# floatingtrees/video-VAE

Measured on AMD Instinct MI355X. Metric: video frames/sec (fwd+bwd) at Bx3x16x256x256, higher is better.
Workload: dtype bf16; 1 GPU; C3: full VideoVAE (enc 9 / dec 12 FactoredAttention + 3D-conv UNet) train step, B=4/GPU x 3x16x256x256, bf16 compute, fp32 params, recon+KL loss, clip+Adam; flavour=model, params=170631304, global_batch=4, frames_per_clip=16, parallelism=dp1, launch_mode=hipgraph(fwd+bwd) + eager all-reduce/clip/Adam

## Files before the change

### include/vvae_hip.h

```cpp
#ifndef VVAE_HIP_H
#define VVAE_HIP_H
#include <stddef.h>
#include <stdint.h>

#ifdef __cplusplus
extern "C" {
#endif

#define VVAE_DT_F32 0
#define VVAE_DT_BF16 1
#define VVAE_ERR_BAD_ARG 1001
#define VVAE_ERR_WORKSPACE 1002
#define VVAE_ERR_LIBRARY 1003

size_t vvae_conv3d_workspace_bytes(int N, int T, int H, int W, int Cin, int Cout, int kt, int kh, int kw, int dtype,
                                   int which );
int vvae_conv3d_fwd(const void* x, int ldx, const float* w, const float* bias, void* y, int ldy,
                    int N, int T, int H, int W, int Cin, int Cout, int kt, int kh, int kw, int dtype,
                    void* ws, size_t ws_bytes, void* stream);
int vvae_conv3d_dgrad(const void* dy, int lddy, const float* w, void* dx, int lddx,
                      int N, int T, int H, int W, int Cin, int Cout, int kt, int kh, int kw, int dtype,
                      void* ws, size_t ws_bytes, void* stream);
int vvae_conv3d_wgrad(const void* x, int ldx, const void* dy, int lddy, float* dw, float* dbias,
                      int N, int T, int H, int W, int Cin, int Cout, int kt, int kh, int kw, int dtype,
                      void* ws, size_t ws_bytes, void* stream);
void vvae_conv3d_force_generic(int on);
int vvae_conv3d_fwd_generic(const void* x, int ldx, const float* w, const float* bias, void* y, int ldy,
                            int N, int T, int H, int W, int Cin, int Cout, int kt, int kh, int kw, int dtype, void* stream);
int vvae_conv3d_dgrad_generic(const void* dy, int lddy, const float* w, void* dx, int lddx,
                              int N, int T, int H, int W, int Cin, int Cout, int kt, int kh, int kw, int dtype, void* stream);
size_t vvae_conv3d_wgrad_generic_ws_bytes(int N, int T, int H, int W, int Cin, int Cout, int kt, int kh, int kw);
int vvae_conv3d_wgrad_generic(const void* x, int ldx, const void* dy, int lddy, float* dw, float* dbias,
                              int N, int T, int H, int W, int Cin, int Cout, int kt, int kh, int kw, int dtype,
                              void* ws, size_t ws_bytes, void* stream);
int vvae_conv3d_deep_config(int on);
int vvae_conv3d_roll_config(int on, int tchunk);
int vvae_conv3d_wgrad_config(int cob16, int blocks);
int vvae_conv3d_bf16_supported(int Cin, int Cout, int kt, int kh, int kw, int ld_in, int ld_out, int which, int flags);
size_t vvae_conv3d_bf16_ws_bytes(int N, int T, int H, int W, int Cin, int Cout, int kt, int kh, int kw, int which);
int vvae_conv3d_pack_bf16(const float* w, void* ws, size_t ws_bytes, int Cin, int Cout, int kt, int kh, int kw,
                          int flags, void* stream);
int vvae_conv3d_pack_grouped_bf16(const float* const* w, void* const* ws, const size_t* ws_bytes, const int* Cin, const int* Cout,
                                  const int* kh, const int* flags, int n, void* stream);
int vvae_conv3d_fwd_bf16(const void* x, int ldx, const float* w, const float* bias, void* y, int ldy,
                         int N, int T, int H, int W, int Cin, int Cout, int kt, int kh, int kw, int flags,
                         int prepacked, void* ws, size_t ws_bytes, void* stream);
int vvae_conv3d_gn_blocks(int N, int T, int H, int W, int Cin, int Cout, int kt, int kh, int kw, int ld_in, int ld_out, int groups);
int vvae_conv3d_fwd_bf16_gn(const void* x, int ldx, const float* w, const float* bias, void* y, int ldy,
                            int N, int T, int H, int W, int Cin, int Cout, int kt, int kh, int kw,
                            int prepacked, void* ws, size_t ws_bytes, float* gn_part, int groups, void* stream);
size_t vvae_conv3d_wgrad_bf16_ws_bytes(int N, int T, int H, int W, int Cin, int Cout, int kt, int kh, int kw);
int vvae_conv3d_wgrad_bf16(const void* x, int ldx, const void* dy, int lddy, float* dw, float* dbias,
                           int N, int T, int H, int W, int Cin, int Cout, int kt, int kh, int kw,
                           void* ws, size_t ws_bytes, void* stream);
int vvae_conv3d_cat2_supported(int Cin, int Cout, int c_split, int kt, int kh, int kw);
int vvae_conv3d_fwd_bf16_cat2(const void* x, int ldx, const void* x2, int ldx2, const float* bias, void* y, int ldy, void* y2, int ldy2,
                              int c_split, int N, int T, int H, int W, int Cin, int Cout, int kt, int kh, int kw, int which,
                              const void* ws, size_t ws_bytes, float* gn_part, int groups, void* stream);
int vvae_conv3d_wgrad_bf16_cat2(const void* x, int ldx, const void* x2, int ldx2, int c_split, const void* dy, int lddy, float* dw,
                                float* dbias, int N, int T, int H, int W, int Cin, int Cout, int kt, int kh, int kw, void* ws,
                                size_t ws_bytes, void* stream);
int vvae_colsum_blocks(long V);
int vvae_colsum(const void* x, int ld, long V, int C, float* out, float* part, int dtype, void* stream);

int vvae_rl_gate_ok(int B2, int T, long per, int LD);
int vvae_rl_gate_blocks(int B2, int T, long per);
int vvae_rl_gate_fwd(const float* z, const float* prob, const float* u, const float* fill, void* comp, float* mask, int B2, int T, long per,
                     int LD, void* stream);
int vvae_rl_gate_bwd(const void* dcomp, const float* mask, float* dz, float* part, int B2, int T, long per, int LD, void* stream);

int vvae_pad_last2_grouped(const float* const* src, float* const* dst, const long* rows, const int* s0, const int* s1, const int* d0,
                           const int* d1, int n, int unpad, void* stream);

int vvae_conv_pointwise_supported(int Cin, int Cout, int kt, int kh, int kw, int ldx, int dtype, const void* x);
size_t vvae_conv_pointwise_ws_bytes(long V, int Cin, int Cout);
int vvae_conv_pointwise_fwd(const void* x, int ldx, const float* w, const float* bias, void* y, int ldy, long V, int Cin, int Cout,
                            int dtype, void* stream);
int vvae_conv_pointwise_fwd_add(const void* x, int ldx, const float* w, const float* bias, const void* addend, int ldadd, void* y, int ldy,
                                long V, int Cin, int Cout, int dtype, void* stream);
int vvae_conv_pointwise_dgrad(const void* dy, int lddy, const float* w, void* dx, int lddx, long V, int Cin, int Cout, int dtype,
                              void* stream);
int vvae_conv_pointwise_dgrad_add(const void* dy, int lddy, const float* w, const void* addend, int ldadd, void* dx, int lddx, long V, int Cin,
                                  int Cout, int dtype, void* stream);
int vvae_conv_pointwise_wgrad(const void* x, int ldx, const void* dy, int lddy, float* dw, float* dbias, long V, int Cin, int Cout,
                              int dtype, void* ws, size_t ws_bytes, void* stream);

int vvae_transpose_grouped_bf16(const void* const* src, void* const* dst, const int* rows, const int* cols, int n, void* stream);

int vvae_loss_tail_plain(const float* mse_ps, int mse_cols, const float* kl_ps, int kl_cols, const float* selection, const float* mask, int B, int T,
                         float max_compression_rate, float magnify_negatives_rate, float gamma1, float gamma2, float* out,
                         float* grads, void* stream);

int vvae_loss_tail_rl(const float* mse, const float* mae, int cols, const float* perc, const float* kl, int kl_cols, const float* sel, const float* act,
                      const float* mask, int B2, int T, float max_compression_rate, float magnify_negatives_rate, float gamma1,
                      float gamma2, float gamma3, float gamma4, float rl_loss_weight, float* out, float* grads, void* stream);

int vvae_encoder_head_ok(int B, int T, int HW, int LD);
int vvae_encoder_head_debug(int flags);
int vvae_encoder_head_fwd(const void* mean, const void* v, const float* w1, const float* b1, const float* w2, const float* b2,
                          const float* u, const float* eps, const float* mask, long mask_pitch, const float* fill, void* logvar,
                          void* comp, float* sel, float* y, float* s1, float* kl_frame, int B, int T, int HW, int LD, void* stream);
int vvae_encoder_head_bwd(const void* mean, const void* v, const void* logvar, const float* eps, const float* mask, long mask_pitch, const float* fill,
                          const float* w1, const float* w2, const float* y, const float* s1, const float* sel, const void* dcomp,
                          const float* dsel, const float* gkl, long gkl_pitch_b, long gkl_pitch_t, const void* dlv_ext, void* dmean, void* dv,
                          float* part1, float* part2, float* part3, float* partb, int B, int T, int HW, int LD, void* stream);

int vvae_encoder_head_eval_fwd(const void* mean, const void* v, const float* w1, const float* b1, const float* w2, const float* b2,
                               const float* u, const float* mask, long mask_pitch, const float* fill, int rl, void* logvar, void* comp,
                               float* sel, float* prob, int B, int T, int HW, int LD, void* stream);

int vvae_recon_metrics_supported(int H, int W, int C, int x_dtype, int y_dtype);
size_t vvae_recon_metrics_part_floats(int B, int T, int H, int W, int C);
int vvae_recon_metrics_fwd(const void* x, int x_dtype, const void* y, int y_dtype, const float* mask, float* mse, float* psnr, float* ssim,
                           float* part, int B, int T, int H, int W, int C, int clamp, void* stream);
int vvae_recon_metrics_wide_supported(int H, int W, int C, int x_dtype, int y_dtype);
size_t vvae_recon_metrics_wide_part_floats(int B, int T, int H, int W, int C);
int vvae_recon_metrics_wide_fwd(const void* x, int x_dtype, const void* y, int y_dtype, const float* mask, float* mse, float* psnr,
                                float* ssim, float* part, int B, int T, int H, int W, int C, int clamp, void* stream);

int vvae_tile_gather_supported(int H, int W, int C, int S, int overlap);
int vvae_tile_gather_u8(const void* src, const float* lut, float* dst, int N, int T, int H, int W, int C, int S, int overlap, int ny, int nx,
                        int first, int count, void* stream);
int vvae_tile_blend_supported(int H, int W, int C, int S, int overlap, int dtype);
int vvae_tile_blend(const void* tiles, int dtype, float* out, int N, int T, int H, int W, int C, int S, int overlap, int ny, int nx,
                    void* stream);
int vvae_window_blend_supported(int L, int frames, int t_overlap, int H, int W, int C, int S, int overlap, int dtype);
int vvae_window_blend(const void* tiles, int dtype, int ring, float* out, int L, int frames, int t_overlap, int n_windows, int f_lo, int f_hi,
                      int H, int W, int C, int S, int overlap, int ny, int nx, void* stream);
int vvae_temporal_mse_supported(int H, int W, int C, int x_dtype, int y_dtype);
size_t vvae_temporal_mse_part_floats(int B, int T, int H, int W, int C);
int vvae_temporal_mse_fwd(const void* x, int x_dtype, const void* y, int y_dtype, float* tmse, float* part, int B, int T, int H, int W, int C,
                          int clamp, void* stream);
int vvae_scene_hist_supported(int H, int W, int hist_size, int space);
size_t vvae_scene_hist_part_bytes(int L, int H, int W, int hist_size, int space);
int vvae_scene_hist_fwd(const void* clip, const int* tabs, unsigned* counts, double* corr, void* part, int L, int H, int W, int hist_size,
                        int space, void* stream);
int vvae_scene_hist_corr(const unsigned* counts, double* corr, int L, int bins, void* stream);
int vvae_crop_resize_supported(int H, int W, int C, int crop_h, int crop_w, int out_h, int out_w);
int vvae_crop_resize_u8(const uint8_t* src, uint8_t* dst, int n, int H, int W, int C, int top, int left, int crop_h, int crop_w, int out_h,
                        int out_w, void* stream);
int vvae_latent_quantise_supported(int hw, int ld, int dtype);
int vvae_latent_quantise(void* latent, int dtype, const float* keep, int8_t* codes, float* step, unsigned* counts, int frames, int hw, int ld,
                         int bits, int dequantise, void* stream);

int vvae_encoder_head_rl_fwd(const void* mean, const void* v, const float* w1, const float* b1, const float* w2, const float* b2,
                             const float* u2, const float* eps, const float* mask, long mask_pitch, const float* fill, void* logvar2,
                             void* mean2, void* comp2, float* prob, float* mask2, float* y, float* s1, float* kl_frame2, int B, int T, int HW,
                             int LD, void* stream);
int vvae_encoder_head_rl_bwd(const void* mean, const void* v, const void* logvar2, const float* eps, const float* mask, long mask_pitch,
                             const float* fill, const float* w1, const float* w2, const float* y, const float* s1, const float* mask2,
                             const void* dcomp2, const float* dprob2, const float* gkl, long gkl_pitch_b, long gkl_pitch_t, const void* dlv_ext,
                             void* dmean, void* dv, float* part1, float* part2, float* part3, float* partb, int B, int T, int HW, int LD,
                             void* stream);

int vvae_silu_bf16(const void* x, void* y, long n, void* stream);

int vvae_linear_residual_bf16(const void* x, int ldx, const void* w, int ldw, const void* bias, int bias_dtype, const void* res, int ldr,
                              void* y, int ldy, int M, int N, int K, void* ws, size_t ws_bytes, void* stream);
int vvae_linear_residual_wt_bf16(const void* x, int ldx, const void* wt, int ldwt, const void* bias, int bias_dtype, const void* res, int ldr,
                                 void* y, int ldy, int M, int N, int K, void* ws, size_t ws_bytes, void* stream);
int vvae_linear_residual_algo(int idx);

int vvae_unpatch_pad_fwd(const void* x, void* y, long frames, int h, int w, int p, int cu, int c, int dtype, void* stream);
int vvae_unpatch_pad_bwd(const void* g, void* gx, long frames, int h, int w, int p, int cu, int c, int dtype, void* stream);

size_t vvae_gn_part_floats(int N, long S, int C);
int vvae_gn_stats(const void* x, int ldx, int N, long S, int C, int G, double* sums, float* part, int dtype, void* stream);
int vvae_gn_finalize(const float* part, int N, int nblk, int G, double* sums, void* stream);
int vvae_gn_silu_fwd(const void* x, int ldx, void* y, int ldy, const double* sums, const float* gamma, const float* beta,
                     int N, long S, int C, int G, float eps, int dtype, void* stream);
int vvae_gn_silu_pool_supported(int H, int W, int C, int G, int ldx, int ldy, int ldp, int dtype);
int vvae_gn_silu_pool_fwd(const void* x, int ldx, void* y, int ldy, void* pool, int ldp, const double* sums, const float* gamma,
                          const float* beta, int N, int T, int H, int W, int C, int G, float eps, int dtype, void* stream);
int vvae_gn_silu_bwd(const void* x, int ldx, const void* dy, int lddy, void* dx, int lddx, const double* sums,
                     const float* gamma, const float* beta, double* csum , float* part,
                     float* dgamma, float* dbeta, int N, long S, int C, int G, float eps, int dtype, void* stream);

int vvae_maxpool_1x2x2_fwd(const void* x, int ldx, void* y, int ldy, int NT, int H, int W, int C, int dtype, void* stream);
int vvae_maxpool_1x2x2_bwd(const void* x, int ldx, const void* dpool, int lddp, const void* dskip, int ldds,
                           void* dx, int lddx, int NT, int H, int W, int C, int dtype, void* stream);

int vvae_convt_1x2x2_fwd(const void* x, int ldx, const float* w, const float* bias, void* y, int ldy,
                         int NT, int H, int W, int Cin, int Cout, int dtype, void* stream);
int vvae_convt_1x2x2_dgrad(const void* dy, int lddy, const float* w, void* dx, int lddx,
                           int NT, int H, int W, int Cin, int Cout, int dtype, void* stream);
size_t vvae_convt_1x2x2_wgrad_ws_bytes(int NT, int H, int W, int Cin, int Cout);
int vvae_convt_1x2x2_wgrad(const void* x, int ldx, const void* dy, int lddy, float* dw,
                           int NT, int H, int W, int Cin, int Cout, int dtype, void* ws, size_t ws_bytes, void* stream);
int vvae_convt_wgrad_bf16_supported(int Cin, int Cout, int ldx, int lddy);
size_t vvae_convt_wgrad_bf16_ws_bytes(int NT, int H, int W, int Cin, int Cout);
int vvae_convt_1x2x2_wgrad_bf16(const void* x, int ldx, const void* dy, int lddy, float* dw, float* dbias, int NT, int H, int W,
                                int Cin, int Cout, void* ws, size_t ws_bytes, void* stream);
int vvae_convt_bf16_supported(int Cin, int Cout, int ld_in, int ld_out);
size_t vvae_convt_bf16_ws_bytes(int Cin, int Cout);
int vvae_convt_1x2x2_bf16(const void* x, int ldx, const float* w, const float* bias, void* y, int ldy,
                          int NT, int H, int W, int Cin, int Cout, int dgrad, void* ws, size_t ws_bytes, void* stream);
int vvae_convt_pack_grouped_bf16(const float* const* w, void* const* ws, const int* Cin, const int* Cout, const int* dgrad, int n, void* stream);

int vvae_temporal_attn_fwd(const void* qkv, int ld, void* out, int ldo, const float* q_scale, const float* k_scale,
                           const float* cos_table, const float* sin_table, const uint8_t* mask, int mask_div,
                           int A, int T, int heads, int D, float eps, int dtype, void* stream);
size_t vvae_temporal_attn_bwd_ws_bytes(int A, int heads, int D);
int vvae_temporal_attn_bwd(const void* qkv, int ld, const void* dout, int lddo, void* dqkv, int lddq,
                           const float* q_scale, const float* k_scale, const float* cos_table, const float* sin_table,
                           const uint8_t* mask, int mask_div, float* dq_scale, float* dk_scale,
                           int A, int T, int heads, int D, float eps, int dtype, void* ws, size_t ws_bytes, void* stream);

int vvae_temporal_attn_fast_supported(int T, int D, int ld, int ldo, int dtype);
int vvae_temporal_attn_fast_blocks(int A, int T, int heads, int D, int dtype);
int vvae_temporal_attn_mfma_enable(int on);
int vvae_temporal_attn_mfma32_enable(int on);
int vvae_temporal_attn_fwd_fast(const void* qkv, int ld, void* out, int ldo, float* lse, const float* q_scale,
                                const float* k_scale, const float* cos_table, const float* sin_table, const uint8_t* mask,
                                int mask_div, int inner, int A, int T, int heads, int D, float eps, int dtype, void* stream);
int vvae_temporal_attn_bwd_fast(const void* qkv, int ld, const void* out, int ldo, const void* dout, int lddo, const float* lse,
                                void* dqkv, int lddq, const float* q_scale, const float* k_scale, const float* cos_table,
                                const float* sin_table, const uint8_t* mask, int mask_div, int inner, float* dscale_part,
                                int A, int T, int heads, int D, float eps, int dtype, void* stream);

int vvae_qk_prep_supported(int D, int dtype);
int vvae_qk_prep_blocks(long tokens, int heads, int D);
int vvae_qk_prep_fwd(const void* qkv, int ld, void* out, int ldo, const float* q_scale, const float* k_scale,
                     const float* cos_table, const float* sin_table, long tokens, int S, int heads, int D, float eps,
                     int dtype, void* stream);
int vvae_qk_prep_bwd(const void* qkv, int ld, const void* dq, long dq_ts, long dq_hs, const void* dk, long dk_ts, long dk_hs,
                     const void* dv, long dv_ts, long dv_hs, void* dqkv, int lddq, const float* q_scale, const float* k_scale,
                     const float* cos_table, const float* sin_table, float* part, long tokens, int S, int heads, int D,
                     float eps, int dtype, void* stream);

int vvae_spatial_attn_supported(int S, int D, int dtype);
int vvae_spatial_attn_fwd(const void* qkv, int ld, void* out, int ldo, float* lse2, const float* q_scale, const float* k_scale,
                          const float* cos_table, const float* sin_table, int A, int S, int heads, int D, float eps, int dtype,
                          void* stream);
int vvae_spatial_attn_bwd(const void* qkv, int ld, const void* out, int ldo, const void* dout, int lddo, const float* lse2,
                          void* dqkv, int lddq, const float* q_scale, const float* k_scale, const float* cos_table,
                          const float* sin_table, float* part, int A, int S, int heads, int D, float eps, int dtype, void* stream);

int vvae_layernorm_supported(int C, int dtype);
int vvae_layernorm_bwd_blocks(long rows, int C, int dtype);
int vvae_delay_us(int us, void* stream);
int vvae_layernorm_fwd_config(int fwd_cap);
int vvae_gn_config(int stream_blocks);
int vvae_layernorm_config(int bwd_cap);
int vvae_layernorm_fwd_mode(int late_stage);
int vvae_layernorm_fwd(const void* x, void* y, const float* gamma, const float* beta, float* mean, float* rstd,
                       const void* addend, void* xsum, long rows, int C, int inner, long outer_pitch, long inner_pitch, float eps,
                       int dtype, void* stream);
int vvae_layernorm_bwd(const void* x, const void* dy, const float* gamma, const float* mean, const float* rstd, const void* dres,
                       void* dx, float* part, long rows, int C, int inner, long outer_pitch, long inner_pitch, int dtype,
                       void* stream);

size_t vvae_loss_part_floats(int B, long M);
int vvae_reparam_kl_fwd(const void* mean, const void* logvar, const float* eps, const float* mask, float* z, float* kl,
                        float* part, int B, int T, long per, int dtype, void* stream);
int vvae_reparam_kl_bwd(const void* mean, const void* logvar, const float* eps, const float* mask, const float* dz,
                        const float* gkl, void* dmean, void* dlogvar, int B, int T, long per, int dtype, void* stream);

int vvae_masked_mse_mae_fwd(const void* video, const void* recon, const float* mask, float* mse, float* mae,
                            float* part, int B, int T, long P, int video_div, int dtype, void* stream);
int vvae_masked_mse_mae_bwd(const void* video, const void* recon, const float* mask, const float* gmse, const float* gmae,
                            void* drecon, int B, int T, long P, int video_div, int dtype, void* stream);

int vvae_gemm_tn_supported(int M, int N, int K, int lda, int ldb);
size_t vvae_gemm_tn_ws_bytes(int M, int N, int K);
int vvae_gemm_tn_bf16(const void* A, int lda, const void* B, int ldb, float* C, float* db, int M, int N, int K,
                      void* ws, size_t ws_bytes, void* stream);
int vvae_gemm_tn_grouped_bf16(const void* const* A, const int* lda, const void* const* B, const int* ldb, float* const* C,
                              float* const* db, const int* M, const int* N, int n, int K, void* stream);
int vvae_gemm_tn_use_big_tiles(int on);

int vvae_sqnorm_blocks(long n);
int vvae_sqnorm_partials(const float* g, long n, double* part, void* stream);
int vvae_adam_clip_step(float* p, const float* g, float* m, float* v, void* p_bf16, long n, const double* gnorm_part, int nparts,
                        double* gnorm_sq_out, float gscale, float max_norm, float lr, float b1, float b2, float eps, long count,
                        void* stream);
int vvae_adam_clip_ema_step(float* p, const float* g, float* m, float* v, void* p_bf16, long n, const double* gnorm_part, int nparts,
                            double* gnorm_sq_out, float gscale, float max_norm, float lr, float b1, float b2, float eps, long count,
                            float* ema, float ema_decay, void* stream);
int vvae_grad_fold_f32(float* dst, const float* src, long n, int overwrite, void* stream);
int vvae_sqnorm_partials2(const float* g, const float* acc, long n, double* part, void* stream);
int vvae_adam_clip_acc_step(float* p, const float* g, const float* acc, float* m, float* v, void* p_bf16, long n,
                            const double* gnorm_part, int nparts, double* gnorm_sq_out, float gscale, float max_norm, float lr, float b1,
                            float b2, float eps, long count, float* ema, float ema_decay, void* stream);
int vvae_swap_refresh_f32(float* a, float* b, void* a_bf16, long n, void* stream);
int vvae_cast_f32_to_bf16(const float* x, void* y, long n, void* stream);
int vvae_gemm_nt_supported(int M, int N, int K, int lda, int ldb, int ldc);
int vvae_gemm_nt_bf16(const void* A, int lda, const void* B, int ldb, void* C, int ldc, const float* bias, const void* res,
                      int ldr, void* C2, int ldc2, int epi, int M, int N, int K, void* stream);
int vvae_gemm_pp_supported(int M, int N, int K, int lda, int ldb, int ldc);
int vvae_gemm_pp_bf16(const void* A, int lda, const void* B, int ldb, void* C, int ldc, const float* bias, const void* res,
                      int ldr, void* C2, int ldc2, int epi, int M, int N, int K, void* stream);
int vvae_gemm_pp_ablate(int bits);
int vvae_gemm_pp_final_ring(int on);
int vvae_gemm_nt_stagger(int units);
int vvae_gemm_nt_persistent(int on);
int vvae_gemm_nt_prefetch(int dist);
int vvae_gemm_nt_prefetch_mask(int mask);

int vvae_sum_rows(const float* part, int rows, int cols, float* out, void* stream);
int vvae_fold_rows_grouped(const void* const* part, float* const* d0, float* const* d1, const int* rows, const int* cols,
                           const int* n0, int n, void* stream);
int vvae_copy_grouped(const float* const* src, float* const* dst, const long* count, int n, void* stream);

int vvae_selftest_xor_lane(const float* x, float* y, double* yd, int n, int o, void* stream);

#ifdef __cplusplus
}
#endif
#endif
```

### video_vae_amd/csrc/attn_temporal_mfma.hip

```cpp
#include "common.hpp"

namespace tmfma {

typedef __bf16 bf16x8 __attribute__((ext_vector_type(8)));
typedef short s16x4v __attribute__((ext_vector_type(4)));

constexpr int T = 16, D = 64;
constexpr int PITCH = 160;
constexpr int IMG = T * PITCH;

struct Dims { int A, heads, mask_div, inner; float eps; long items; };

__device__ __forceinline__ long token_of(const Dims& d, int a, int row) {
    return (long)(a / d.inner) * T * d.inner + (long)row * d.inner + (a % d.inner);
}

__device__ __forceinline__ void unpack8(const uint4& r, float* v) {
    const uint32_t w[4] = {r.x, r.y, r.z, r.w};
#pragma unroll
    for (int i = 0; i < 4; ++i) { v[2 * i] = __uint_as_float(w[i] << 16); v[2 * i + 1] = __uint_as_float(w[i] & 0xffff0000u); }
}
__device__ __forceinline__ uint4 pack8(const float* v) {
    uint32_t w[4];
#pragma unroll
    for (int i = 0; i < 4; ++i) w[i] = (uint32_t)f2bf(v[2 * i]) | ((uint32_t)f2bf(v[2 * i + 1]) << 16);
    return make_uint4(w[0], w[1], w[2], w[3]);
}
__device__ __forceinline__ bf16x8 frag8(const uint4& r) { return __builtin_bit_cast(bf16x8, r); }
__device__ __forceinline__ s16x4v pack4(float a, float b, float c, float e) {
    s16x4v r = {(short)f2bf(a), (short)f2bf(b), (short)f2bf(c), (short)f2bf(e)};
    return r;
}
__device__ __forceinline__ s16x4v tr4(const unsigned char* p) {
    typedef __attribute__((address_space(3))) s16x4v* lds_ptr;
    return __builtin_amdgcn_ds_read_tr16_b64_v4i16((lds_ptr)p);
}
__device__ __forceinline__ f32x4 mfma32(const bf16x8& a, const bf16x8& b, f32x4 c) { return __builtin_amdgcn_mfma_f32_16x16x32_bf16(a, b, c, 0, 0, 0); }
__device__ __forceinline__ f32x4 mfma16(const s16x4v& a, const s16x4v& b, f32x4 c) { return __builtin_amdgcn_mfma_f32_16x16x16bf16_1k(a, b, c, 0, 0, 0); }

__device__ __forceinline__ float psum(float v) { return butterfly_sum<32, 16>(v); }
__device__ __forceinline__ float pmax(float v) { v = fmaxf(v, xor_lane<32>(v)); return fmaxf(v, xor_lane<16>(v)); }

__device__ __forceinline__ float xhat16(float (&x)[16], float eps) {
    float s = 0.f, ss = 0.f;
#pragma unroll
    for (int i = 0; i < 16; ++i) { s += x[i]; ss += x[i] * x[i]; }
    s = psum(s); ss = psum(ss);
    const float mean = s * (1.f / D);
    float var = ss * (1.f / D) - mean * mean;
    var = var < 0.f ? 0.f : var;
    const float rstd = rsqrtf(var + eps);
#pragma unroll
    for (int i = 0; i < 16; ++i) x[i] = (x[i] - mean) * rstd;
    return rstd;
}
__device__ __forceinline__ void ln_rope16(float (&x)[16], const float* __restrict__ sc, float eps, const float* __restrict__ cs,
                                          const float* __restrict__ sn) {
    xhat16(x, eps);
#pragma unroll
    for (int i = 0; i < 8; ++i) {
        float lo = x[i] * sc[i], hi = x[i + 8] * sc[i + 8];
        round2<bf16_t>(lo, hi);
        float a = lo * cs[i], b = -hi * sn[i], c = hi * cs[i + 8], e = lo * sn[i + 8];
        round2<bf16_t>(a, b);
        round2<bf16_t>(c, e);
        float y0 = a + b, y1 = c + e;
        round2<bf16_t>(y0, y1);
        x[i] = y0; x[i + 8] = y1;
    }
}
__device__ __forceinline__ void tab16(const float* __restrict__ row, int p, float (&r)[16]) {
    const float4* lo = reinterpret_cast<const float4*>(row + 8 * p);
    const float4* hi = reinterpret_cast<const float4*>(row + 32 + 8 * p);
    const float4 a = lo[0], b = lo[1], c = hi[0], e = hi[1];
    r[0] = a.x; r[1] = a.y; r[2] = a.z; r[3] = a.w; r[4] = b.x; r[5] = b.y; r[6] = b.z; r[7] = b.w;
    r[8] = c.x; r[9] = c.y; r[10] = c.z; r[11] = c.w; r[12] = e.x; r[13] = e.y; r[14] = e.z; r[15] = e.w;
}
__device__ __forceinline__ void norm_row(const bf16_t* __restrict__ g, int p, const float (&sc)[16], float eps, const float (&cs)[16],
                                         const float (&sn)[16], uint4& f0, uint4& f1) {
    float x[16];
    unpack8(*reinterpret_cast<const uint4*>(g + 8 * p), x);
    unpack8(*reinterpret_cast<const uint4*>(g + 32 + 8 * p), x + 8);
    ln_rope16(x, sc, eps, cs, sn);
    f0 = pack8(x); f1 = pack8(x + 8);
}
__device__ __forceinline__ void put_row(unsigned char* img, int t, int p, const uint4& f0, const uint4& f1) {
    *reinterpret_cast<uint4*>(img + t * PITCH + 16 * p) = f0;
    *reinterpret_cast<uint4*>(img + t * PITCH + 64 + 16 * p) = f1;
}
__device__ __forceinline__ void wave_lds_fence() {
    __builtin_amdgcn_wave_barrier();
    __builtin_amdgcn_s_waitcnt(0xc07f);
    __builtin_amdgcn_wave_barrier();
}
__device__ __forceinline__ s16x4v tr_rows(const unsigned char* img, int p, int i, int tile) {
    return tr4(img + (4 * p + (i >> 2)) * PITCH + 32 * tile + 8 * (i & 3));
}

__global__ __launch_bounds__(256) void tattn16_fwd_mfma(const bf16_t* __restrict__ qkv, int ld, bf16_t* __restrict__ out, int ldo,
                                                       float* __restrict__ lse, const float* __restrict__ q_scale,
                                                       const float* __restrict__ k_scale, const float* __restrict__ cosT,
                                                       const float* __restrict__ sinT, const uint8_t* __restrict__ mask, Dims d)
{
    __shared__ __attribute__((aligned(16))) unsigned char smem[4 * IMG];
    const int lane = threadIdx.x & 63, wave = threadIdx.x >> 6;
    const int t = lane & 15, p = lane >> 4;
    const long item = (long)blockIdx.x * 4 + wave;
    if (item >= d.items) return;
    const int a = (int)(item / d.heads), h = (int)(item % d.heads);
    const int HD = d.heads * D;
    const long tok = token_of(d, a, t);
    const bf16_t* g = qkv + tok * ld + h * D;
    unsigned char* vimg = smem + wave * IMG;

    const uint4 vlo = *reinterpret_cast<const uint4*>(g + 2 * HD + 8 * p);
    const uint4 vhi = *reinterpret_cast<const uint4*>(g + 2 * HD + 32 + 8 * p);
    float cs[16], sn[16], sc[16];
    tab16(cosT + t * D, p, cs);
    tab16(sinT + t * D, p, sn);
    uint4 q0, q1, k0, k1;
    tab16(q_scale, p, sc);
    norm_row(g, p, sc, d.eps, cs, sn, q0, q1);
    tab16(k_scale, p, sc);
    norm_row(g + HD, p, sc, d.eps, cs, sn, k0, k1);
    put_row(vimg, t, p, vlo, vhi);

    f32x4 s = {0.f, 0.f, 0.f, 0.f};
    s = mfma32(frag8(k0), frag8(q0), s);
    s = mfma32(frag8(k1), frag8(q1), s);
    const float scale = 0.125f;
    uint32_t mk = 0x01010101u;
    if (mask) mk = *reinterpret_cast<const uint32_t*>(mask + (long)(a / d.mask_div) * T + 4 * p);
    float e[4];
    float m = -3.0e38f;
#pragma unroll
    for (int r = 0; r < 4; ++r) {
        e[r] = ((mk >> (8 * r)) & 0xff) ? s[r] * scale : -3.0e38f;
        m = fmaxf(m, e[r]);
    }
    m = pmax(m);
    float l = 0.f;
#pragma unroll
    for (int r = 0; r < 4; ++r) { e[r] = ((mk >> (8 * r)) & 0xff) ? __expf(e[r] - m) : 0.f; l += e[r]; }
    l = psum(l);
    const float inv = l > 0.f ? 1.f / l : 0.f;
    const s16x4v pf = pack4(e[0] * inv, e[1] * inv, e[2] * inv, e[3] * inv);
    if (p == 0) lse[item * T + t] = l > 0.f ? m + __logf(l) : 0.f;

    wave_lds_fence();
    bf16_t* o = out + tok * ldo + h * D + 4 * p;
#pragma unroll
    for (int tile = 0; tile < 4; ++tile) {
        f32x4 acc = {0.f, 0.f, 0.f, 0.f};
        acc = mfma16(tr_rows(vimg, p, t, tile), pf, acc);
        const s16x4v ob = pack4(acc[0], acc[1], acc[2], acc[3]);
        *reinterpret_cast<uint2*>(o + 16 * tile) = __builtin_bit_cast(uint2, ob);
    }
}

__device__ __forceinline__ void rope_ln_bwd_cols(float (&g)[4][4], const float (&raw)[4][4], int p, int frame, float eps,
                                                 const float* __restrict__ scale, const float* __restrict__ cosT,
                                                 const float* __restrict__ sinT, float (&contrib)[4][4])
{
    float xh[4][4];
    float s = 0.f, ss = 0.f;
#pragma unroll
    for (int tl = 0; tl < 4; ++tl)
#pragma unroll
        for (int r = 0; r < 4; ++r) { s += raw[tl][r]; ss += raw[tl][r] * raw[tl][r]; }
    s = psum(s); ss = psum(ss);
    const float mean = s * (1.f / D);
    float var = ss * (1.f / D) - mean * mean;
    var = var < 0.f ? 0.f : var;
    const float rstd = rsqrtf(var + eps);
#pragma unroll
    for (int tl = 0; tl < 4; ++tl)
#pragma unroll
        for (int r = 0; r < 4; ++r) xh[tl][r] = (raw[tl][r] - mean) * rstd;
    const float* cr = cosT + frame * D;
    const float* sr = sinT + frame * D;
#pragma unroll
    for (int tl = 0; tl < 2; ++tl) {
        const float4 cl = *reinterpret_cast<const float4*>(cr + 16 * tl + 4 * p), ch = *reinterpret_cast<const float4*>(cr + 32 + 16 * tl + 4 * p);
        const float4 sl = *reinterpret_cast<const float4*>(sr + 16 * tl + 4 * p), sh = *reinterpret_cast<const float4*>(sr + 32 + 16 * tl + 4 * p);
        const float c_lo[4] = {cl.x, cl.y, cl.z, cl.w}, c_hi[4] = {ch.x, ch.y, ch.z, ch.w};
        const float s_lo[4] = {sl.x, sl.y, sl.z, sl.w}, s_hi[4] = {sh.x, sh.y, sh.z, sh.w};
#pragma unroll
        for (int r = 0; r < 4; ++r) {
            const float lo = g[tl][r], hi = g[tl + 2][r];
            g[tl][r] = lo * c_lo[r] + hi * s_hi[r];
            g[tl + 2][r] = hi * c_hi[r] - lo * s_lo[r];
        }
    }
    float s1 = 0.f, s2 = 0.f;
    float scv[4][4];
#pragma unroll
    for (int tl = 0; tl < 4; ++tl) {
        const float4 v = *reinterpret_cast<const float4*>(scale + 16 * tl + 4 * p);
        scv[tl][0] = v.x; scv[tl][1] = v.y; scv[tl][2] = v.z; scv[tl][3] = v.w;
#pragma unroll
        for (int r = 0; r < 4; ++r) { const float dxh = g[tl][r] * scv[tl][r]; s1 += dxh; s2 += dxh * xh[tl][r]; }
    }
    s1 = psum(s1) * (1.f / D); s2 = psum(s2) * (1.f / D);
#pragma unroll
    for (int tl = 0; tl < 4; ++tl)
#pragma unroll
        for (int r = 0; r < 4; ++r) {
            const float dy = g[tl][r], x = xh[tl][r];
            g[tl][r] = rstd * (dy * scv[tl][r] - s1 - x * s2);
            contrib[tl][r] = dy * x;
        }
}

__device__ __forceinline__ void load_cols(const bf16_t* __restrict__ row, int p, float (&v)[4][4]) {
#pragma unroll
    for (int tl = 0; tl < 4; ++tl) {
        const uint2 u = *reinterpret_cast<const uint2*>(row + 16 * tl + 4 * p);
        v[tl][0] = __uint_as_float(u.x << 16); v[tl][1] = __uint_as_float(u.x & 0xffff0000u);
        v[tl][2] = __uint_as_float(u.y << 16); v[tl][3] = __uint_as_float(u.y & 0xffff0000u);
    }
}
__device__ __forceinline__ void store_cols(bf16_t* __restrict__ row, int p, const float (&v)[4][4]) {
#pragma unroll
    for (int tl = 0; tl < 4; ++tl) {
        const s16x4v b = pack4(v[tl][0], v[tl][1], v[tl][2], v[tl][3]);
        *reinterpret_cast<uint2*>(row + 16 * tl + 4 * p) = __builtin_bit_cast(uint2, b);
    }
}

__global__ __launch_bounds__(256, 4) void tattn16_bwd_mfma(const bf16_t* __restrict__ qkv, int ld, const bf16_t* __restrict__ out, int ldo,
                                                          const bf16_t* __restrict__ dout, int lddo, const float* __restrict__ lse,
                                                          bf16_t* __restrict__ dqkv, int lddq, const float* __restrict__ q_scale,
                                                          const float* __restrict__ k_scale, const float* __restrict__ cosT,
                                                          const float* __restrict__ sinT, const uint8_t* __restrict__ mask,
                                                          float* __restrict__ part, Dims d)
{
    __shared__ __attribute__((aligned(16))) unsigned char smem[4 * (3 * IMG + 64)];
    const int lane = threadIdx.x & 63, wave = threadIdx.x >> 6;
    const int t = lane & 15, p = lane >> 4;
    unsigned char* base = smem + wave * (3 * IMG + 64);
    unsigned char* kimg = base;
    unsigned char* qimg = base + IMG;
    unsigned char* gimg = base + 2 * IMG;
    float* dlds = reinterpret_cast<float*>(base + 3 * IMG);
    const int HD = d.heads * D;
    const float scale = 0.125f;
    float accq[4][4], acck[4][4];
#pragma unroll
    for (int tl = 0; tl < 4; ++tl)
#pragma unroll
        for (int r = 0; r < 4; ++r) { accq[tl][r] = 0.f; acck[tl][r] = 0.f; }

    const long item = (long)blockIdx.x * 4 + wave;
    if (item < d.items) {
        const float* ct = cosT; const float* st_ = sinT; const float* qsp = q_scale; const float* ksp = k_scale;
        const int a = (int)(item / d.heads), h = (int)(item % d.heads);
        const long tok = token_of(d, a, t);
        const bf16_t* g = qkv + tok * ld + h * D;
        uint4 q0, q1, k0, k1;
        {
            float cs[16], sn[16], sc[16];
            tab16(ct + t * D, p, cs);
            tab16(st_ + t * D, p, sn);
            tab16(qsp, p, sc);
            norm_row(g, p, sc, d.eps, cs, sn, q0, q1);
            tab16(ksp, p, sc);
            norm_row(g + HD, p, sc, d.eps, cs, sn, k0, k1);
        }
        const uint4 v0 = *reinterpret_cast<const uint4*>(g + 2 * HD + 8 * p), v1 = *reinterpret_cast<const uint4*>(g + 2 * HD + 32 + 8 * p);
        const bf16_t* go = dout + tok * lddo + h * D;
        const uint4 g0 = *reinterpret_cast<const uint4*>(go + 8 * p), g1 = *reinterpret_cast<const uint4*>(go + 32 + 8 * p);
        const bf16_t* oo = out + tok * ldo + h * D;
        float delta;
        {
            float a16[16], b16[16];
            unpack8(g0, a16); unpack8(g1, a16 + 8);
            unpack8(*reinterpret_cast<const uint4*>(oo + 8 * p), b16); unpack8(*reinterpret_cast<const uint4*>(oo + 32 + 8 * p), b16 + 8);
            float s = 0.f;
#pragma unroll
            for (int i = 0; i < 16; ++i) s += a16[i] * b16[i];
            delta = psum(s);
        }
        wave_lds_fence();
        put_row(kimg, t, p, k0, k1);
        put_row(qimg, t, p, q0, q1);
        put_row(gimg, t, p, g0, g1);
        if (p == 0) dlds[t] = delta;
        const float lse_q = lse[item * T + t];
        uint32_t mk = 0x01010101u, mcol = 1u;
        if (mask) {
            const uint8_t* mrow = mask + (long)(a / d.mask_div) * T;
            mk = *reinterpret_cast<const uint32_t*>(mrow + 4 * p);
            mcol = mrow[t];
        }
        bf16_t* dg = dqkv + tok * lddq + h * D;
        s16x4v dsf, pf, dsf2;
        {
            f32x4 st = {0.f, 0.f, 0.f, 0.f}, dpt = {0.f, 0.f, 0.f, 0.f}, sq = {0.f, 0.f, 0.f, 0.f}, dp = {0.f, 0.f, 0.f, 0.f};
            st = mfma32(frag8(k0), frag8(q0), st);
            st = mfma32(frag8(k1), frag8(q1), st);
            dpt = mfma32(frag8(v0), frag8(g0), dpt);
            dpt = mfma32(frag8(v1), frag8(g1), dpt);
            sq = mfma32(frag8(q0), frag8(k0), sq);
            sq = mfma32(frag8(q1), frag8(k1), sq);
            dp = mfma32(frag8(g0), frag8(v0), dp);
            dp = mfma32(frag8(g1), frag8(v1), dp);
            float dst[4];
#pragma unroll
            for (int r = 0; r < 4; ++r) {
                const float pr = ((mk >> (8 * r)) & 0xff) ? __expf(st[r] * scale - lse_q) : 0.f;
                dst[r] = pr * (dpt[r] - delta) * scale;
            }
            dsf = pack4(dst[0], dst[1], dst[2], dst[3]);
            wave_lds_fence();
            const float4 lse4 = *reinterpret_cast<const float4*>(lse + item * T + 4 * p);
            const float4 del4 = *reinterpret_cast<const float4*>(dlds + 4 * p);
            const float lq[4] = {lse4.x, lse4.y, lse4.z, lse4.w}, dl[4] = {del4.x, del4.y, del4.z, del4.w};
            float pq[4], dsq[4];
#pragma unroll
            for (int r = 0; r < 4; ++r) {
                const float pr = mcol ? __expf(sq[r] * scale - lq[r]) : 0.f;
                pq[r] = pr;
                dsq[r] = pr * (dp[r] - dl[r]) * scale;
            }
            pf = pack4(pq[0], pq[1], pq[2], pq[3]);
            dsf2 = pack4(dsq[0], dsq[1], dsq[2], dsq[3]);
        }
        {
            float dq[4][4];
#pragma unroll
            for (int tile = 0; tile < 4; ++tile) {
                f32x4 acc = {0.f, 0.f, 0.f, 0.f};
                acc = mfma16(tr_rows(kimg, p, t, tile), dsf, acc);
#pragma unroll
                for (int r = 0; r < 4; ++r) dq[tile][r] = acc[r];
            }
            float raw[4][4], contrib[4][4];
            load_cols(g, p, raw);
            rope_ln_bwd_cols(dq, raw, p, t, d.eps, qsp, ct, st_, contrib);
            store_cols(dg, p, dq);
#pragma unroll
            for (int tl = 0; tl < 4; ++tl)
#pragma unroll
                for (int r = 0; r < 4; ++r) accq[tl][r] += contrib[tl][r];
        }
        {
            float dv[4][4];
#pragma unroll
            for (int tile = 0; tile < 4; ++tile) {
                f32x4 a1 = {0.f, 0.f, 0.f, 0.f};
                a1 = mfma16(tr_rows(gimg, p, t, tile), pf, a1);
#pragma unroll
                for (int r = 0; r < 4; ++r) dv[tile][r] = a1[r];
            }
            store_cols(dg + 2 * HD, p, dv);
        }
        {
            float dk[4][4];
#pragma unroll
            for (int tile = 0; tile < 4; ++tile) {
                f32x4 a2 = {0.f, 0.f, 0.f, 0.f};
                a2 = mfma16(tr_rows(qimg, p, t, tile), dsf2, a2);
#pragma unroll
                for (int r = 0; r < 4; ++r) dk[tile][r] = a2[r];
            }
            float raw[4][4], contrib[4][4];
            load_cols(g + HD, p, raw);
            rope_ln_bwd_cols(dk, raw, p, t, d.eps, ksp, ct, st_, contrib);
            store_cols(dg + HD, p, dk);
#pragma unroll
            for (int tl = 0; tl < 4; ++tl)
#pragma unroll
                for (int r = 0; r < 4; ++r) acck[tl][r] += contrib[tl][r];
        }
    }
    __syncthreads();
    float* red = reinterpret_cast<float*>(smem);
#pragma unroll
    for (int tl = 0; tl < 4; ++tl)
#pragma unroll
        for (int r = 0; r < 4; ++r) {
            const float a = butterfly_sum<8, 1>(accq[tl][r]), b = butterfly_sum<8, 1>(acck[tl][r]);
            if (t == 0) { red[wave * 2 * D + 16 * tl + 4 * p + r] = a; red[wave * 2 * D + D + 16 * tl + 4 * p + r] = b; }
        }
    __syncthreads();
    if (threadIdx.x < 2 * D)
        part[(long)blockIdx.x * 2 * D + threadIdx.x] = (red[threadIdx.x] + red[2 * D + threadIdx.x]) + (red[4 * D + threadIdx.x] + red[6 * D + threadIdx.x]);
}

int g_enable = 1;

inline int bwd_blocks(long items) { return (int)((items + 3) / 4); }

bool shape_ok(int T_, int D_, int ld, int ldo, int dtype) {
    return g_enable && dtype == VVAE_DT_BF16 && T_ == T && D_ == D && ld % 8 == 0 && ldo % 8 == 0;
}

}

extern "C" int vvae_temporal_attn_mfma_enable(int on)
{
    tmfma::g_enable = on ? 1 : 0;
    return 0;
}

int tmfma_supported(int T, int D, int ld, int ldo, int dtype) { return tmfma::shape_ok(T, D, ld, ldo, dtype) ? 1 : 0; }
int tmfma_bwd_rows(long items) { return tmfma::bwd_blocks(items); }

int tmfma_fwd(const void* qkv, int ld, void* out, int ldo, float* lse, const float* qs, const float* ks, const float* cosT, const float* sinT,
              const uint8_t* mask, int mask_div, int inner, int A, int heads, float eps, hipStream_t s)
{
    tmfma::Dims d{A, heads, mask_div, inner, eps, (long)A * heads};
    if (mask && ((uintptr_t)mask % 4)) return VVAE_ERR_BAD_ARG;
    hipLaunchKernelGGL(tmfma::tattn16_fwd_mfma, dim3((unsigned)((d.items + 3) / 4)), dim3(256), 0, s, (const bf16_t*)qkv, ld, (bf16_t*)out, ldo, lse,
                       qs, ks, cosT, sinT, mask, d);
    VVAE_LAUNCH_CHECK();
    return 0;
}

int tmfma_bwd(const void* qkv, int ld, const void* out, int ldo, const void* dout, int lddo, const float* lse, void* dqkv, int lddq,
              const float* qs, const float* ks, const float* cosT, const float* sinT, const uint8_t* mask, int mask_div, int inner,
              float* part, int A, int heads, float eps, hipStream_t s)
{
    tmfma::Dims d{A, heads, mask_div, inner, eps, (long)A * heads};
    if (mask && ((uintptr_t)mask % 4)) return VVAE_ERR_BAD_ARG;
    hipLaunchKernelGGL(tmfma::tattn16_bwd_mfma, dim3((unsigned)tmfma::bwd_blocks(d.items)), dim3(256), 0, s, (const bf16_t*)qkv, ld,
                       (const bf16_t*)out, ldo, (const bf16_t*)dout, lddo, lse, (bf16_t*)dqkv, lddq, qs, ks, cosT, sinT, mask, part, d);
    VVAE_LAUNCH_CHECK();
    return 0;
}
```

Before: 2012 frames/s.

## Make temporal attention MFMA kernels persistent with software-prefetched item loads

Converts the forward and backward 16-frame temporal attention kernels into grid-stride persistent loops capped at 512 blocks. Each wave prefetches the next item's q/k/v and mask while computing the current one, and hoists cos/sin and scale tables out of the per-item loop. This aims to hide global load latency and cut block launch and setup overhead. It also drops one intermediate bf16 rounding in the RoPE output, which changes numerics slightly. Ablation variants compiled under a macro are added for probing.

New measurement: 2034 frames/s, median of 6. +1.1%, better.

```diff
diff --git a/include/vvae_hip.h b/include/vvae_hip.h
--- a/include/vvae_hip.h
+++ b/include/vvae_hip.h
@@ -209,6 +209,7 @@
 int vvae_temporal_attn_fast_supported(int T, int D, int ld, int ldo, int dtype);
 int vvae_temporal_attn_fast_blocks(int A, int T, int heads, int D, int dtype);
 int vvae_temporal_attn_mfma_enable(int on);
+int vvae_temporal_attn_mfma_config(int fwd_cap, int bwd_cap);
 int vvae_temporal_attn_mfma32_enable(int on);
 int vvae_temporal_attn_fwd_fast(const void* qkv, int ld, void* out, int ldo, float* lse, const float* q_scale,
                                 const float* k_scale, const float* cos_table, const float* sin_table, const uint8_t* mask,
diff --git a/video_vae_amd/csrc/attn_temporal_mfma.hip b/video_vae_amd/csrc/attn_temporal_mfma.hip
--- a/video_vae_amd/csrc/attn_temporal_mfma.hip
+++ b/video_vae_amd/csrc/attn_temporal_mfma.hip
@@ -8,12 +8,11 @@
 constexpr int T = 16, D = 64;
 constexpr int PITCH = 160;
 constexpr int IMG = T * PITCH;
+constexpr int BWD_WAVE_LDS = 5 * IMG + 128;
+
+constexpr int ABL_LOAD = 1, ABL_MATH = 2, ABL_MFMA = 4, ABL_STORE = 8;
 
 struct Dims { int A, heads, mask_div, inner; float eps; long items; };
-
-__device__ __forceinline__ long token_of(const Dims& d, int a, int row) {
-    return (long)(a / d.inner) * T * d.inner + (long)row * d.inner + (a % d.inner);
-}
 
 __device__ __forceinline__ void unpack8(const uint4& r, float* v) {
     const uint32_t w[4] = {r.x, r.y, r.z, r.w};
@@ -35,8 +34,27 @@
     typedef __attribute__((address_space(3))) s16x4v* lds_ptr;
     return __builtin_amdgcn_ds_read_tr16_b64_v4i16((lds_ptr)p);
 }
-__device__ __forceinline__ f32x4 mfma32(const bf16x8& a, const bf16x8& b, f32x4 c) { return __builtin_amdgcn_mfma_f32_16x16x32_bf16(a, b, c, 0, 0, 0); }
-__device__ __forceinline__ f32x4 mfma16(const s16x4v& a, const s16x4v& b, f32x4 c) { return __builtin_amdgcn_mfma_f32_16x16x16bf16_1k(a, b, c, 0, 0, 0); }
+template <int ABL> __device__ __forceinline__ f32x4 mfma32(const uint4& a, const uint4& b, f32x4 c) {
+    if constexpr (ABL & ABL_MFMA) { c[0] += __uint_as_float(((a.x ^ b.x) & 0x007fffffu) | 0x3f000000u); return c; }
+    else return __builtin_amdgcn_mfma_f32_16x16x32_bf16(frag8(a), frag8(b), c, 0, 0, 0);
+}
+template <int ABL> __device__ __forceinline__ f32x4 mfma16(const s16x4v& a, const s16x4v& b, f32x4 c) {
+    if constexpr (ABL & ABL_MFMA) {
+        const uint2 x = __builtin_bit_cast(uint2, a), y = __builtin_bit_cast(uint2, b);
+        c[0] += __uint_as_float(((x.x ^ y.x) & 0x007fffffu) | 0x3f000000u);
+        c[1] += __uint_as_float(((x.y ^ y.y) & 0x007fffffu) | 0x3f000000u);
+        return c;
+    } else return __builtin_amdgcn_mfma_f32_16x16x16bf16_1k(a, b, c, 0, 0, 0);
+}
+template <int ABL> __device__ __forceinline__ uint4 ld16(const bf16_t* __restrict__ p, const bf16_t* __restrict__ line) {
+    if constexpr (ABL & ABL_LOAD) return *reinterpret_cast<const uint4*>(line);
+    else return *reinterpret_cast<const uint4*>(p);
+}
+template <int ABL> __device__ __forceinline__ void st8(bf16_t* __restrict__ p, const s16x4v& v) {
+    const uint2 u = __builtin_bit_cast(uint2, v);
+    if constexpr (ABL & ABL_STORE) { if (u.x == 0x7fc17fc2u && u.y == 0x7fc37fc4u) *reinterpret_cast<uint2*>(p) = u; }
+    else *reinterpret_cast<uint2*>(p) = u;
+}
 
 __device__ __forceinline__ float psum(float v) { return butterfly_sum<32, 16>(v); }
 __device__ __forceinline__ float pmax(float v) { v = fmaxf(v, xor_lane<32>(v)); return fmaxf(v, xor_lane<16>(v)); }
@@ -54,8 +72,7 @@
     for (int i = 0; i < 16; ++i) x[i] = (x[i] - mean) * rstd;
     return rstd;
 }
-__device__ __forceinline__ void ln_rope16(float (&x)[16], const float* __restrict__ sc, float eps, const float* __restrict__ cs,
-                                          const float* __restrict__ sn) {
+__device__ __forceinline__ void ln_rope16(float (&x)[16], const float (&sc)[16], float eps, const float (&cs)[16], const float (&sn)[16]) {
     xhat16(x, eps);
 #pragma unroll
     for (int i = 0; i < 8; ++i) {
@@ -64,9 +81,7 @@
         float a = lo * cs[i], b = -hi * sn[i], c = hi * cs[i + 8], e = lo * sn[i + 8];
         round2<bf16_t>(a, b);
         round2<bf16_t>(c, e);
-        float y0 = a + b, y1 = c + e;
-        round2<bf16_t>(y0, y1);
-        x[i] = y0; x[i + 8] = y1;
+        x[i] = a + b; x[i + 8] = c + e;
     }
 }
 __device__ __forceinline__ void tab16(const float* __restrict__ row, int p, float (&r)[16]) {
@@ -76,13 +91,16 @@
     r[0] = a.x; r[1] = a.y; r[2] = a.z; r[3] = a.w; r[4] = b.x; r[5] = b.y; r[6] = b.z; r[7] = b.w;
     r[8] = c.x; r[9] = c.y; r[10] = c.z; r[11] = c.w; r[12] = e.x; r[13] = e.y; r[14] = e.z; r[15] = e.w;
 }
-__device__ __forceinline__ void norm_row(const bf16_t* __restrict__ g, int p, const float (&sc)[16], float eps, const float (&cs)[16],
-                                         const float (&sn)[16], uint4& f0, uint4& f1) {
-    float x[16];
-    unpack8(*reinterpret_cast<const uint4*>(g + 8 * p), x);
-    unpack8(*reinterpret_cast<const uint4*>(g + 32 + 8 * p), x + 8);
-    ln_rope16(x, sc, eps, cs, sn);
-    f0 = pack8(x); f1 = pack8(x + 8);
+template <int ABL> __device__ __forceinline__ void norm_row(const uint4& lo, const uint4& hi, const float (&sc)[16], float eps,
+                                                            const float (&cs)[16], const float (&sn)[16], uint4& f0, uint4& f1) {
+    if constexpr (ABL & ABL_MATH) { f0 = lo; f1 = hi; }
+    else {
+        float x[16];
+        unpack8(lo, x);
+        unpack8(hi, x + 8);
+        ln_rope16(x, sc, eps, cs, sn);
+        f0 = pack8(x); f1 = pack8(x + 8);
+    }
 }
 __device__ __forceinline__ void put_row(unsigned char* img, int t, int p, const uint4& f0, const uint4& f1) {
     *reinterpret_cast<uint4*>(img + t * PITCH + 16 * p) = f0;
@@ -93,74 +111,141 @@
     __builtin_amdgcn_s_waitcnt(0xc07f);
     __builtin_amdgcn_wave_barrier();
 }
+__device__ __forceinline__ void drain_loads() { __builtin_amdgcn_s_waitcnt(0x0f70); }
 __device__ __forceinline__ s16x4v tr_rows(const unsigned char* img, int p, int i, int tile) {
     return tr4(img + (4 * p + (i >> 2)) * PITCH + 32 * tile + 8 * (i & 3));
 }
 
-__global__ __launch_bounds__(256) void tattn16_fwd_mfma(const bf16_t* __restrict__ qkv, int ld, bf16_t* __restrict__ out, int ldo,
-                                                       float* __restrict__ lse, const float* __restrict__ q_scale,
-                                                       const float* __restrict__ k_scale, const float* __restrict__ cosT,
-                                                       const float* __restrict__ sinT, const uint8_t* __restrict__ mask, Dims d)
-{
-    __shared__ __attribute__((aligned(16))) unsigned char smem[4 * IMG];
-    const int lane = threadIdx.x & 63, wave = threadIdx.x >> 6;
+struct ItemAt { int a, h; long tok0; };
+__device__ __forceinline__ ItemAt item_at(const Dims& d, long item) {
+    const unsigned it = (unsigned)item, hd = (unsigned)d.heads, in = (unsigned)d.inner;
+    const unsigned a = it / hd, h = it - a * hd;
+    const unsigned ao = a / in, ai = a - ao * in;
+    return ItemAt{(int)a, (int)h, (long)ao * T * d.inner + ai};
+}
+
+struct FwdRaw { uint4 q0, q1, k0, k1, v0, v1; uint32_t mk; };
+
+template <int ABL> __device__ __forceinline__ void fwd_load(FwdRaw& r, const bf16_t* __restrict__ qkv, int ld, const uint8_t* __restrict__ mask,
+                                                            const Dims& d, long item, long lane_in, int p, const bf16_t* __restrict__ line) {
+    const ItemAt at = item_at(d, item);
+    const int HD = d.heads * D;
+    const bf16_t* g = qkv + at.tok0 * ld + at.h * D + lane_in;
+    r.q0 = ld16<ABL>(g, line); r.q1 = ld16<ABL>(g + 32, line);
+    r.k0 = ld16<ABL>(g + HD, line); r.k1 = ld16<ABL>(g + HD + 32, line);
+    r.v0 = ld16<ABL>(g + 2 * HD, line); r.v1 = ld16<ABL>(g + 2 * HD + 32, line);
+    r.mk = 0x01010101u;
+    if (mask) r.mk = *reinterpret_cast<const uint32_t*>(mask + (long)(at.a / d.mask_div) * T + 4 * p);
+}
+
+template <int ABL> __device__ __forceinline__ void fwd_item(const FwdRaw& r, long item, unsigned char* vimg, bf16_t* __restrict__ o,
+                                                            float* __restrict__ lse, int t, int p, float eps, const float (&cs)[16],
+                                                            const float (&sn)[16], const float (&scq)[16], const float (&sck)[16]) {
+    uint4 q0, q1, k0, k1;
+    norm_row<ABL>(r.q0, r.q1, scq, eps, cs, sn, q0, q1);
+    norm_row<ABL>(r.k0, r.k1, sck, eps, cs, sn, k0, k1);
+    wave_lds_fence();
+    put_row(vimg, t, p, r.v0, r.v1);
+
+    f32x4 s = {0.f, 0.f, 0.f, 0.f};
+    s = mfma32<ABL>(k0, q0, s);
+    s = mfma32<ABL>(k1, q1, s);
+    const float scale = 0.125f;
+    const uint32_t mk = r.mk;
+    s16x4v pf;
+    float lse_v;
+    if constexpr (ABL & ABL_MATH) {
+        pf = pack4(s[0], s[1], s[2], s[3]);
+        lse_v = s[0] + __uint_as_float(mk);
+    } else {
+        float e[4];
+        float m = -3.0e38f;
+#pragma unroll
+        for (int r_ = 0; r_ < 4; ++r_) {
+            e[r_] = ((mk >> (8 * r_)) & 0xff) ? s[r_] * scale : -3.0e38f;
+            m = fmaxf(m, e[r_]);
+        }
+        m = pmax(m);
+        float l = 0.f;
+#pragma unroll
+        for (int r_ = 0; r_ < 4; ++r_) { e[r_] = ((mk >> (8 * r_)) & 0xff) ? __expf(e[r_] - m) : 0.f; l += e[r_]; }
+        l = psum(l);
+        const float inv = l > 0.f ? 1.f / l : 0.f;
+        pf = pack4(e[0] * inv, e[1] * inv, e[2] * inv, e[3] * inv);
+        lse_v = l > 0.f ? m + __logf(l) : 0.f;
+    }
+    if (p == 0) {
+        if constexpr (ABL & ABL_STORE) { if (lse_v == -1.2345e-30f) lse[item * T + t] = lse_v; }
+        else lse[item * T + t] = lse_v;
+    }
+
+    wave_lds_fence();
+#pragma unroll
+    for (int tile = 0; tile < 4; ++tile) {
+        f32x4 acc = {0.f, 0.f, 0.f, 0.f};
+        acc = mfma16<ABL>(tr_rows(vimg, p, t, tile), pf, acc);
+        st8<ABL>(o + 16 * tile, pack4(acc[0], acc[1], acc[2], acc[3]));
+    }
+}
+
+template <int ABL> __device__ __forceinline__ void fwd_walk(const bf16_t* __restrict__ qkv, int ld, bf16_t* __restrict__ out, int ldo,
+                                                            float* __restrict__ lse, const float* __restrict__ q_scale,
+                                                            const float* __restrict__ k_scale, const float* __restrict__ cosT,
+                                                            const float* __restrict__ sinT, const uint8_t* __restrict__ mask, const Dims& d,
+                                                            unsigned char* smem)
+{
+    const int lane = threadIdx.x & 63, wave = __builtin_amdgcn_readfirstlane(threadIdx.x >> 6);
     const int t = lane & 15, p = lane >> 4;
-    const long item = (long)blockIdx.x * 4 + wave;
+    const long stride = (long)gridDim.x * 4;
+    long item = (long)blockIdx.x * 4 + wave;
     if (item >= d.items) return;
-    const int a = (int)(item / d.heads), h = (int)(item % d.heads);
-    const int HD = d.heads * D;
-    const long tok = token_of(d, a, t);
-    const bf16_t* g = qkv + tok * ld + h * D;
     unsigned char* vimg = smem + wave * IMG;
-
-    const uint4 vlo = *reinterpret_cast<const uint4*>(g + 2 * HD + 8 * p);
-    const uint4 vhi = *reinterpret_cast<const uint4*>(g + 2 * HD + 32 + 8 * p);
-    float cs[16], sn[16], sc[16];
+    float cs[16], sn[16], scq[16], sck[16];
     tab16(cosT + t * D, p, cs);
     tab16(sinT + t * D, p, sn);
-    uint4 q0, q1, k0, k1;
-    tab16(q_scale, p, sc);
-    norm_row(g, p, sc, d.eps, cs, sn, q0, q1);
-    tab16(k_scale, p, sc);
-    norm_row(g + HD, p, sc, d.eps, cs, sn, k0, k1);
-    put_row(vimg, t, p, vlo, vhi);
-
-    f32x4 s = {0.f, 0.f, 0.f, 0.f};
-    s = mfma32(frag8(k0), frag8(q0), s);
-    s = mfma32(frag8(k1), frag8(q1), s);
-    const float scale = 0.125f;
-    uint32_t mk = 0x01010101u;
-    if (mask) mk = *reinterpret_cast<const uint32_t*>(mask + (long)(a / d.mask_div) * T + 4 * p);
-    float e[4];
-    float m = -3.0e38f;
-#pragma unroll
-    for (int r = 0; r < 4; ++r) {
-        e[r] = ((mk >> (8 * r)) & 0xff) ? s[r] * scale : -3.0e38f;
-        m = fmaxf(m, e[r]);
-    }
-    m = pmax(m);
-    float l = 0.f;
-#pragma unroll
-    for (int r = 0; r < 4; ++r) { e[r] = ((mk >> (8 * r)) & 0xff) ? __expf(e[r] - m) : 0.f; l += e[r]; }
-    l = psum(l);
-    const float inv = l > 0.f ? 1.f / l : 0.f;
-    const s16x4v pf = pack4(e[0] * inv, e[1] * inv, e[2] * inv, e[3] * inv);
-    if (p == 0) lse[item * T + t] = l > 0.f ? m + __logf(l) : 0.f;
-
-    wave_lds_fence();
-    bf16_t* o = out + tok * ldo + h * D + 4 * p;
-#pragma unroll
-    for (int tile = 0; tile < 4; ++tile) {
-        f32x4 acc = {0.f, 0.f, 0.f, 0.f};
-        acc = mfma16(tr_rows(vimg, p, t, tile), pf, acc);
-        const s16x4v ob = pack4(acc[0], acc[1], acc[2], acc[3]);
-        *reinterpret_cast<uint2*>(o + 16 * tile) = __builtin_bit_cast(uint2, ob);
-    }
-}
-
-__device__ __forceinline__ void rope_ln_bwd_cols(float (&g)[4][4], const float (&raw)[4][4], int p, int frame, float eps,
-                                                 const float* __restrict__ scale, const float* __restrict__ cosT,
-                                                 const float* __restrict__ sinT, float (&contrib)[4][4])
+    tab16(q_scale, p, scq);
+    tab16(k_scale, p, sck);
+    const long lane_in = (long)t * d.inner * ld + 8 * p;
+    const long lane_out = (long)t * d.inner * ldo + 4 * p;
+    const bf16_t* line = qkv + 8 * (lane & 7);
+    FwdRaw cur;
+    fwd_load<ABL>(cur, qkv, ld, mask, d, item, lane_in, p, line);
+    drain_loads();
+    for (;;) {
+        const long nxt = item + stride;
+        const bool more = nxt < d.items;
+        FwdRaw nx;
+        if (more) fwd_load<ABL>(nx, qkv, ld, mask, d, nxt, lane_in, p, line);
+        const ItemAt at = item_at(d, item);
+        fwd_item<ABL>(cur, item, vimg, out + at.tok0 * ldo + at.h * D + lane_out, lse, t, p, d.eps, cs, sn, scq, sck);
+        if (!more) break;
+        cur = nx; item = nxt;
+    }
+}
+
+__global__ __launch_bounds__(256, 2) void tattn16_fwd_mfma(const bf16_t* __restrict__ qkv, int ld, bf16_t* __restrict__ out, int ldo,
+                                                          float* __restrict__ lse, const float* __restrict__ q_scale,
+                                                          const float* __restrict__ k_scale, const float* __restrict__ cosT,
+                                                          const float* __restrict__ sinT, const uint8_t* __restrict__ mask, Dims d)
+{
+    __shared__ __attribute__((aligned(16))) unsigned char smem[4 * IMG];
+    fwd_walk<0>(qkv, ld, out, ldo, lse, q_scale, k_scale, cosT, sinT, mask, d, smem);
+}
+
+struct ColTabs { float c_lo[2][4], c_hi[2][4], s_lo[2][4], s_hi[2][4]; };
+__device__ __forceinline__ void col_tabs(const float* __restrict__ cr, const float* __restrict__ sr, int p, ColTabs& ct) {
+#pragma unroll
+    for (int tl = 0; tl < 2; ++tl) {
+        const float4 cl = *reinterpret_cast<const float4*>(cr + 16 * tl + 4 * p), ch = *reinterpret_cast<const float4*>(cr + 32 + 16 * tl + 4 * p);
+        const float4 sl = *reinterpret_cast<const float4*>(sr + 16 * tl + 4 * p), sh = *reinterpret_cast<const float4*>(sr + 32 + 16 * tl + 4 * p);
+        ct.c_lo[tl][0] = cl.x; ct.c_lo[tl][1] = cl.y; ct.c_lo[tl][2] = cl.z; ct.c_lo[tl][3] = cl.w;
+        ct.c_hi[tl][0] = ch.x; ct.c_hi[tl][1] = ch.y; ct.c_hi[tl][2] = ch.z; ct.c_hi[tl][3] = ch.w;
+        ct.s_lo[tl][0] = sl.x; ct.s_lo[tl][1] = sl.y; ct.s_lo[tl][2] = sl.z; ct.s_lo[tl][3] = sl.w;
+        ct.s_hi[tl][0] = sh.x; ct.s_hi[tl][1] = sh.y; ct.s_hi[tl][2] = sh.z; ct.s_hi[tl][3] = sh.w;
+    }
+}
+__device__ __forceinline__ void rope_ln_bwd_cols(float (&g)[4][4], const float (&raw)[4][4], int p, float eps, const float* scale,
+                                                 const ColTabs& ct, float (&acc)[4][4])
 {
     float xh[4][4];
     float s = 0.f, ss = 0.f;
@@ -177,19 +262,13 @@
     for (int tl = 0; tl < 4; ++tl)
 #pragma unroll
         for (int r = 0; r < 4; ++r) xh[tl][r] = (raw[tl][r] - mean) * rstd;
-    const float* cr = cosT + frame * D;
-    const float* sr = sinT + frame * D;
 #pragma unroll
     for (int tl = 0; tl < 2; ++tl) {
-        const float4 cl = *reinterpret_cast<const float4*>(cr + 16 * tl + 4 * p), ch = *reinterpret_cast<const float4*>(cr + 32 + 16 * tl + 4 * p);
-        const float4 sl = *reinterpret_cast<const float4*>(sr + 16 * tl + 4 * p), sh = *reinterpret_cast<const float4*>(sr + 32 + 16 * tl + 4 * p);
-        const float c_lo[4] = {cl.x, cl.y, cl.z, cl.w}, c_hi[4] = {ch.x, ch.y, ch.z, ch.w};
-        const float s_lo[4] = {sl.x, sl.y, sl.z, sl.w}, s_hi[4] = {sh.x, sh.y, sh.z, sh.w};
 #pragma unroll
         for (int r = 0; r < 4; ++r) {
             const float lo = g[tl][r], hi = g[tl + 2][r];
-            g[tl][r] = lo * c_lo[r] + hi * s_hi[r];
-            g[tl + 2][r] = hi * c_hi[r] - lo * s_lo[r];
+            g[tl][r] = lo * ct.c_lo[tl][r] + hi * ct.s_hi[tl][r];
+            g[tl + 2][r] = hi * ct.c_hi[tl][r] - lo * ct.s_lo[tl][r];
         }
     }
     float s1 = 0.f, s2 = 0.f;
@@ -208,189 +287,274 @@
         for (int r = 0; r < 4; ++r) {
             const float dy = g[tl][r], x = xh[tl][r];
             g[tl][r] = rstd * (dy * scv[tl][r] - s1 - x * s2);
-            contrib[tl][r] = dy * x;
-        }
-}
-
-__device__ __forceinline__ void load_cols(const bf16_t* __restrict__ row, int p, float (&v)[4][4]) {
+            acc[tl][r] += dy * x;
+        }
+}
+
+__device__ __forceinline__ void load_cols(const unsigned char* img, int i, int p, float (&v)[4][4]) {
 #pragma unroll
     for (int tl = 0; tl < 4; ++tl) {
-        const uint2 u = *reinterpret_cast<const uint2*>(row + 16 * tl + 4 * p);
+        const uint2 u = *reinterpret_cast<const uint2*>(img + i * PITCH + 32 * tl + 8 * p);
         v[tl][0] = __uint_as_float(u.x << 16); v[tl][1] = __uint_as_float(u.x & 0xffff0000u);
         v[tl][2] = __uint_as_float(u.y << 16); v[tl][3] = __uint_as_float(u.y & 0xffff0000u);
     }
 }
-__device__ __forceinline__ void store_cols(bf16_t* __restrict__ row, int p, const float (&v)[4][4]) {
-#pragma unroll
-    for (int tl = 0; tl < 4; ++tl) {
-        const s16x4v b = pack4(v[tl][0], v[tl][1], v[tl][2], v[tl][3]);
-        *reinterpret_cast<uint2*>(row + 16 * tl + 4 * p) = __builtin_bit_cast(uint2, b);
-    }
-}
-
-__global__ __launch_bounds__(256, 4) void tattn16_bwd_mfma(const bf16_t* __restrict__ qkv, int ld, const bf16_t* __restrict__ out, int ldo,
+template <int ABL> __device__ __forceinline__ void store_cols(bf16_t* __restrict__ row, const float (&v)[4][4]) {
+#pragma unroll
+    for (int tl = 0; tl < 4; ++tl) st8<ABL>(row + 16 * tl, pack4(v[tl][0], v[tl][1], v[tl][2], v[tl][3]));
+}
+
+struct BwdRaw { uint4 q0, q1, k0, k1, v0, v1, g0, g1, o0, o1; float lse_q; uint32_t mk, mcol; };
+
+template <int ABL> __device__ __forceinline__ void bwd_load(BwdRaw& r, const bf16_t* __restrict__ qkv, int ld, const bf16_t* __restrict__ out,
+                                                            int ldo, const bf16_t* __restrict__ dout, int lddo, const float* __restrict__ lse,
+                                                            const uint8_t* __restrict__ mask, const Dims& d, long item, int t, int p,
+                                                            const bf16_t* __restrict__ line) {
+    const ItemAt at = item_at(d, item);
+    const int HD = d.heads * D;
+    const long row = (long)t * d.inner;
+    const bf16_t* g = qkv + (at.tok0 + row) * ld + at.h * D + 8 * p;
+    const bf16_t* go = dout + (at.tok0 + row) * lddo + at.h * D + 8 * p;
+    const bf16_t* oo = out + (at.tok0 + row) * ldo + at.h * D + 8 * p;
+    r.q0 = ld16<ABL>(g, line); r.q1 = ld16<ABL>(g + 32, line);
+    r.k0 = ld16<ABL>(g + HD, line); r.k1 = ld16<ABL>(g + HD + 32, line);
+    r.v0 = ld16<ABL>(g + 2 * HD, line); r.v1 = ld16<ABL>(g + 2 * HD + 32, line);
+    r.g0 = ld16<ABL>(go, line); r.g1 = ld16<ABL>(go + 32, line);
+    r.o0 = ld16<ABL>(oo, line); r.o1 = ld16<ABL>(oo + 32, line);
+    r.lse_q = lse[item * T + t];
+    r.mk = 0x01010101u; r.mcol = 1u;
+    if (mask) {
+        const uint8_t* mrow = mask + (long)(at.a / d.mask_div) * T;
+        r.mk = *reinterpret_cast<const uint32_t*>(mrow + 4 * p);
+        r.mcol = mrow[t];
+    }
+}
+
+template <int ABL> __device__ __forceinline__ void bwd_item(const BwdRaw& r, unsigned char* base, bf16_t* __restrict__ dg, int HD, int t, int p,
+                                                            float eps, const float (&cs)[16], const float (&sn)[16], const ColTabs& ct,
+                                                            const float* stab, float (&accq)[4][4], float (&acck)[4][4]) {
+    unsigned char* kimg = base;
+    unsigned char* qimg = base + IMG;
+    unsigned char* gimg = base + 2 * IMG;
+    unsigned char* rqimg = base + 3 * IMG;
+    unsigned char* rkimg = base + 4 * IMG;
+    float* dlds = reinterpret_cast<float*>(base + 5 * IMG);
+    const float scale = 0.125f;
+    uint4 q0, q1, k0, k1;
+    {
+        float sc[16];
+        tab16(stab, p, sc);
+        norm_row<ABL>(r.q0, r.q1, sc, eps, cs, sn, q0, q1);
+        tab16(stab + D, p, sc);
+        norm_row<ABL>(r.k0, r.k1, sc, eps, cs, sn, k0, k1);
+    }
+    const uint4 v0 = r.v0, v1 = r.v1, g0 = r.g0, g1 = r.g1;
+    float delta;
+    if constexpr (ABL & ABL_MATH) delta = __uint_as_float((g0.x ^ r.o0.x ^ r.o1.y) & 0x3fffffffu);
+    else {
+        float a16[16], b16[16];
+        unpack8(g0, a16); unpack8(g1, a16 + 8);
+        unpack8(r.o0, b16); unpack8(r.o1, b16 + 8);
+        float s = 0.f;
+#pragma unroll
+        for (int i = 0; i < 16; ++i) s += a16[i] * b16[i];
+        delta = psum(s);
+    }
+    wave_lds_fence();
+    put_row(kimg, t, p, k0, k1);
+    put_row(qimg, t, p, q0, q1);
+    put_row(gimg, t, p, g0, g1);
+    put_row(rqimg, t, p, r.q0, r.q1);
+    put_row(rkimg, t, p, r.k0, r.k1);
+    const float lse_q = r.lse_q;
+    if (p == 0) { dlds[t] = delta; dlds[T + t] = lse_q; }
+    const uint32_t mk = r.mk, mcol = r.mcol;
+    s16x4v dsf, pf, dsf2;
+    {
+        f32x4 st = {0.f, 0.f, 0.f, 0.f}, dpt = {0.f, 0.f, 0.f, 0.f}, sq = {0.f, 0.f, 0.f, 0.f}, dp = {0.f, 0.f, 0.f, 0.f};
+        st = mfma32<ABL>(k0, q0, st);
+        st = mfma32<ABL>(k1, q1, st);
+        dpt = mfma32<ABL>(v0, g0, dpt);
+        dpt = mfma32<ABL>(v1, g1, dpt);
+        sq = mfma32<ABL>(q0, k0, sq);
+        sq = mfma32<ABL>(q1, k1, sq);
+        dp = mfma32<ABL>(g0, v0, dp);
+        dp = mfma32<ABL>(g1, v1, dp);
+        float dst[4];
+#pragma unroll
+        for (int r_ = 0; r_ < 4; ++r_) {
+            if constexpr (ABL & ABL_MATH) dst[r_] = st[r_] + dpt[r_] + delta + lse_q + __uint_as_float(mk);
+            else {
+                const float pr = ((mk >> (8 * r_)) & 0xff) ? __expf(st[r_] * scale - lse_q) : 0.f;
+                dst[r_] = pr * (dpt[r_] - delta) * scale;
+            }
+        }
+        dsf = pack4(dst[0], dst[1], dst[2], dst[3]);
+        wave_lds_fence();
+        const float4 del4 = *reinterpret_cast<const float4*>(dlds + 4 * p);
+        const float4 lse4 = *reinterpret_cast<const float4*>(dlds + T + 4 * p);
+        const float lq[4] = {lse4.x, lse4.y, lse4.z, lse4.w}, dl[4] = {del4.x, del4.y, del4.z, del4.w};
+        float pq[4], dsq[4];
+#pragma unroll
+        for (int r_ = 0; r_ < 4; ++r_) {
+            if constexpr (ABL & ABL_MATH) { pq[r_] = sq[r_] + lq[r_] + __uint_as_float(mcol); dsq[r_] = dp[r_] + dl[r_]; }
+            else {
+                const float pr = mcol ? __expf(sq[r_] * scale - lq[r_]) : 0.f;
+                pq[r_] = pr;
+                dsq[r_] = pr * (dp[r_] - dl[r_]) * scale;
+            }
+        }
+        pf = pack4(pq[0], pq[1], pq[2], pq[3]);
+        dsf2 = pack4(dsq[0], dsq[1], dsq[2], dsq[3]);
+    }
+    {
+        float dq[4][4];
+#pragma unroll
+        for (int tile = 0; tile < 4; ++tile) {
+            f32x4 acc = {0.f, 0.f, 0.f, 0.f};
+            acc = mfma16<ABL>(tr_rows(kimg, p, t, tile), dsf, acc);
+#pragma unroll
+            for (int r_ = 0; r_ < 4; ++r_) dq[tile][r_] = acc[r_];
+        }
+        float raw[4][4];
+        load_cols(rqimg, t, p, raw);
+        if constexpr (ABL & ABL_MATH) {
+#pragma unroll
+            for (int tl = 0; tl < 4; ++tl)
+#pragma unroll
+                for (int r_ = 0; r_ < 4; ++r_) { dq[tl][r_] += raw[tl][r_]; accq[tl][r_] += dq[tl][r_]; }
+        } else rope_ln_bwd_cols(dq, raw, p, eps, stab, ct, accq);
+        store_cols<ABL>(dg, dq);
+    }
+    {
+        float dv[4][4];
+#pragma unroll
+        for (int tile = 0; tile < 4; ++tile) {
+            f32x4 a1 = {0.f, 0.f, 0.f, 0.f};
+            a1 = mfma16<ABL>(tr_rows(gimg, p, t, tile), pf, a1);
+#pragma unroll
+            for (int r_ = 0; r_ < 4; ++r_) dv[tile][r_] = a1[r_];
+        }
+        store_cols<ABL>(dg + 2 * HD, dv);
+    }
+    {
+        float dk[4][4];
+#pragma unroll
+        for (int tile = 0; tile < 4; ++tile) {
+            f32x4 a2 = {0.f, 0.f, 0.f, 0.f};
+            a2 = mfma16<ABL>(tr_rows(qimg, p, t, tile), dsf2, a2);
+#pragma unroll
+            for (int r_ = 0; r_ < 4; ++r_) dk[tile][r_] = a2[r_];
+        }
+        float raw[4][4];
+        load_cols(rkimg, t, p, raw);
+        if constexpr (ABL & ABL_MATH) {
+#pragma unroll
+            for (int tl = 0; tl < 4; ++tl)
+#pragma unroll
+                for (int r_ = 0; r_ < 4; ++r_) { dk[tl][r_] += raw[tl][r_]; acck[tl][r_] += dk[tl][r_]; }
+        } else rope_ln_bwd_cols(dk, raw, p, eps, stab + D, ct, acck);
+        store_cols<ABL>(dg + HD, dk);
+    }
+}
+
+template <int ABL> __device__ __forceinline__ void bwd_walk(const bf16_t* __restrict__ qkv, int ld, const bf16_t* __restrict__ out, int ldo,
+                                                            const bf16_t* __restrict__ dout, int lddo, const float* __restrict__ lse,
+                                                            bf16_t* __restrict__ dqkv, int lddq, const float* __restrict__ q_scale,
+                                                            const float* __restrict__ k_scale, const float* __restrict__ cosT,
+                                                            const float* __restrict__ sinT, const uint8_t* __restrict__ mask,
+                                                            float* __restrict__ part, const Dims& d, unsigned char* smem)
+{
+    const int lane = threadIdx.x & 63, wave = __builtin_amdgcn_readfirstlane(threadIdx.x >> 6);
+    const int t = lane & 15, p = lane >> 4;
+    unsigned char* base = smem + wave * BWD_WAVE_LDS;
+    float* stab = reinterpret_cast<float*>(smem + 4 * BWD_WAVE_LDS);
+    if (threadIdx.x < 2 * D) stab[threadIdx.x] = threadIdx.x < D ? q_scale[threadIdx.x] : k_scale[threadIdx.x - D];
+    __syncthreads();
+    const int HD = d.heads * D;
+    float accq[4][4], acck[4][4];
+#pragma unroll
+    for (int tl = 0; tl < 4; ++tl)
+#pragma unroll
+        for (int r = 0; r < 4; ++r) { accq[tl][r] = 0.f; acck[tl][r] = 0.f; }
+
+    const long stride = (long)gridDim.x * 4;
+    long item = (long)blockIdx.x * 4 + wave;
+    if (item < d.items) {
+        float cs[16], sn[16];
+        ColTabs ct;
+        tab16(cosT + t * D, p, cs);
+        tab16(sinT + t * D, p, sn);
+        col_tabs(cosT + t * D, sinT + t * D, p, ct);
+        const long lane_out = (long)t * d.inner * lddq + 4 * p;
+        const bf16_t* line = qkv + 8 * (lane & 7);
+        BwdRaw cur;
+        bwd_load<ABL>(cur, qkv, ld, out, ldo, dout, lddo, lse, mask, d, item, t, p, line);
+        drain_loads();
+        for (;;) {
+            const long nxt = item + stride;
+            const bool more = nxt < d.items;
+            BwdRaw nx;
+            if (more) bwd_load<ABL>(nx, qkv, ld, out, ldo, dout, lddo, lse, mask, d, nxt, t, p, line);
+            const ItemAt at = item_at(d, item);
+            bwd_item<ABL>(cur, base, dqkv + at.tok0 * lddq + at.h * D + lane_out, HD, t, p, d.eps, cs, sn, ct, stab, accq, acck);
+            if (!more) break;
+            cur = nx; item = nxt;
+        }
+    }
+    __syncthreads();
+    float* red = reinterpret_cast<float*>(smem);
+#pragma unroll
+    for (int tl = 0; tl < 4; ++tl)
+#pragma unroll
+        for (int r = 0; r < 4; ++r) {
+            const float a = butterfly_sum<8, 1>(accq[tl][r]), b = butterfly_sum<8, 1>(acck[tl][r]);
+            if (t == 0) { red[wave * 2 * D + 16 * tl + 4 * p + r] = a; red[wave * 2 * D + D + 16 * tl + 4 * p + r] = b; }
+        }
+    __syncthreads();
+    if (threadIdx.x < 2 * D)
+        part[(long)blockIdx.x * 2 * D + threadIdx.x] = (red[threadIdx.x] + red[2 * D + threadIdx.x]) + (red[4 * D + threadIdx.x] + red[6 * D + threadIdx.x]);
+}
+
+__global__ __launch_bounds__(256, 2) void tattn16_bwd_mfma(const bf16_t* __restrict__ qkv, int ld, const bf16_t* __restrict__ out, int ldo,
                                                           const bf16_t* __restrict__ dout, int lddo, const float* __restrict__ lse,
                                                           bf16_t* __restrict__ dqkv, int lddq, const float* __restrict__ q_scale,
                                                           const float* __restrict__ k_scale, const float* __restrict__ cosT,
                                                           const float* __restrict__ sinT, const uint8_t* __restrict__ mask,
                                                           float* __restrict__ part, Dims d)
 {
-    __shared__ __attribute__((aligned(16))) unsigned char smem[4 * (3 * IMG + 64)];
-    const int lane = threadIdx.x & 63, wave = threadIdx.x >> 6;
-    const int t = lane & 15, p = lane >> 4;
-    unsigned char* base = smem + wave * (3 * IMG + 64);
-    unsigned char* kimg = base;
-    unsigned char* qimg = base + IMG;
-    unsigned char* gimg = base + 2 * IMG;
-    float* dlds = reinterpret_cast<float*>(base + 3 * IMG);
-    const int HD = d.heads * D;
-    const float scale = 0.125f;
-    float accq[4][4], acck[4][4];
-#pragma unroll
-    for (int tl = 0; tl < 4; ++tl)
-#pragma unroll
-        for (int r = 0; r < 4; ++r) { accq[tl][r] = 0.f; acck[tl][r] = 0.f; }
-
-    const long item = (long)blockIdx.x * 4 + wave;
-    if (item < d.items) {
-        const float* ct = cosT; const float* st_ = sinT; const float* qsp = q_scale; const float* ksp = k_scale;
-        const int a = (int)(item / d.heads), h = (int)(item % d.heads);
-        const long tok = token_of(d, a, t);
-        const bf16_t* g = qkv + tok * ld + h * D;
-        uint4 q0, q1, k0, k1;
-        {
-            float cs[16], sn[16], sc[16];
-            tab16(ct + t * D, p, cs);
-            tab16(st_ + t * D, p, sn);
-            tab16(qsp, p, sc);
-            norm_row(g, p, sc, d.eps, cs, sn, q0, q1);
-            tab16(ksp, p, sc);
-            norm_row(g + HD, p, sc, d.eps, cs, sn, k0, k1);
-        }
-        const uint4 v0 = *reinterpret_cast<const uint4*>(g + 2 * HD + 8 * p), v1 = *reinterpret_cast<const uint4*>(g + 2 * HD + 32 + 8 * p);
-        const bf16_t* go = dout + tok * lddo + h * D;
-        const uint4 g0 = *reinterpret_cast<const uint4*>(go + 8 * p), g1 = *reinterpret_cast<const uint4*>(go + 32 + 8 * p);
-        const bf16_t* oo = out + tok * ldo + h * D;
-        float delta;
-        {
-            float a16[16], b16[16];
-            unpack8(g0, a16); unpack8(g1, a16 + 8);
-            unpack8(*reinterpret_cast<const uint4*>(oo + 8 * p), b16); unpack8(*reinterpret_cast<const uint4*>(oo + 32 + 8 * p), b16 + 8);
-            float s = 0.f;
-#pragma unroll
-            for (int i = 0; i < 16; ++i) s += a16[i] * b16[i];
-            delta = psum(s);
-        }
-        wave_lds_fence();
-        put_row(kimg, t, p, k0, k1);
-        put_row(qimg, t, p, q0, q1);
-        put_row(gimg, t, p, g0, g1);
-        if (p == 0) dlds[t] = delta;
-        const float lse_q = lse[item * T + t];
-        uint32_t mk = 0x01010101u, mcol = 1u;
-        if (mask) {
-            const uint8_t* mrow = mask + (long)(a / d.mask_div) * T;
-            mk = *reinterpret_cast<const uint32_t*>(mrow + 4 * p);
-            mcol = mrow[t];
-        }
-        bf16_t* dg = dqkv + tok * lddq + h * D;
-        s16x4v dsf, pf, dsf2;
-        {
-            f32x4 st = {0.f, 0.f, 0.f, 0.f}, dpt = {0.f, 0.f, 0.f, 0.f}, sq = {0.f, 0.f, 0.f, 0.f}, dp = {0.f, 0.f, 0.f, 0.f};
-            st = mfma32(frag8(k0), frag8(q0), st);
-            st = mfma32(frag8(k1), frag8(q1), st);
-            dpt = mfma32(frag8(v0), frag8(g0), dpt);
-            dpt = mfma32(frag8(v1), frag8(g1), dpt);
-            sq = mfma32(frag8(q0), frag8(k0), sq);
-            sq = mfma32(frag8(q1), frag8(k1), sq);
-            dp = mfma32(frag8(g0), frag8(v0), dp);
-            dp = mfma32(frag8(g1), frag8(v1), dp);
-            float dst[4];
-#pragma unroll
-            for (int r = 0; r < 4; ++r) {
-                const float pr = ((mk >> (8 * r)) & 0xff) ? __expf(st[r] * scale - lse_q) : 0.f;
-                dst[r] = pr * (dpt[r] - delta) * scale;
-            }
-            dsf = pack4(dst[0], dst[1], dst[2], dst[3]);
-            wave_lds_fence();
-            const float4 lse4 = *reinterpret_cast<const float4*>(lse + item * T + 4 * p);
-            const float4 del4 = *reinterpret_cast<const float4*>(dlds + 4 * p);
-            const float lq[4] = {lse4.x, lse4.y, lse4.z, lse4.w}, dl[4] = {del4.x, del4.y, del4.z, del4.w};
-            float pq[4], dsq[4];
-#pragma unroll
-            for (int r = 0; r < 4; ++r) {
-                const float pr = mcol ? __expf(sq[r] * scale - lq[r]) : 0.f;
-                pq[r] = pr;
-                dsq[r] = pr * (dp[r] - dl[r]) * scale;
-            }
-            pf = pack4(pq[0], pq[1], pq[2], pq[3]);
-            dsf2 = pack4(dsq[0], dsq[1], dsq[2], dsq[3]);
-        }
-        {
-            float dq[4][4];
-#pragma unroll
-            for (int tile = 0; tile < 4; ++tile) {
-                f32x4 acc = {0.f, 0.f, 0.f, 0.f};
-                acc = mfma16(tr_rows(kimg, p, t, tile), dsf, acc);
-#pragma unroll
-                for (int r = 0; r < 4; ++r) dq[tile][r] = acc[r];
-            }
-            float raw[4][4], contrib[4][4];
-            load_cols(g, p, raw);
-            rope_ln_bwd_cols(dq, raw, p, t, d.eps, qsp, ct, st_, contrib);
-            store_cols(dg, p, dq);
-#pragma unroll
-            for (int tl = 0; tl < 4; ++tl)
-#pragma unroll
-                for (int r = 0; r < 4; ++r) accq[tl][r] += contrib[tl][r];
-        }
-        {
-            float dv[4][4];
-#pragma unroll
-            for (int tile = 0; tile < 4; ++tile) {
-                f32x4 a1 = {0.f, 0.f, 0.f, 0.f};
-                a1 = mfma16(tr_rows(gimg, p, t, tile), pf, a1);
-#pragma unroll
-                for (int r = 0; r < 4; ++r) dv[tile][r] = a1[r];
-            }
-            store_cols(dg + 2 * HD, p, dv);
-        }
-        {
-            float dk[4][4];
-#pragma unroll
-            for (int tile = 0; tile < 4; ++tile) {
-                f32x4 a2 = {0.f, 0.f, 0.f, 0.f};
-                a2 = mfma16(tr_rows(qimg, p, t, tile), dsf2, a2);
-#pragma unroll
-                for (int r = 0; r < 4; ++r) dk[tile][r] = a2[r];
-            }
-            float raw[4][4], contrib[4][4];
-            load_cols(g + HD, p, raw);
-            rope_ln_bwd_cols(dk, raw, p, t, d.eps, ksp, ct, st_, contrib);
-            store_cols(dg + HD, p, dk);
-#pragma unroll
-            for (int tl = 0; tl < 4; ++tl)
-#pragma unroll
-                for (int r = 0; r < 4; ++r) acck[tl][r] += contrib[tl][r];
-        }
-    }
-    __syncthreads();
-    float* red = reinterpret_cast<float*>(smem);
-#pragma unroll
-    for (int tl = 0; tl < 4; ++tl)
-#pragma unroll
-        for (int r = 0; r < 4; ++r) {
-            const float a = butterfly_sum<8, 1>(accq[tl][r]), b = butterfly_sum<8, 1>(acck[tl][r]);
-            if (t == 0) { red[wave * 2 * D + 16 * tl + 4 * p + r] = a; red[wave * 2 * D + D + 16 * tl + 4 * p + r] = b; }
-        }
-    __syncthreads();
-    if (threadIdx.x < 2 * D)
-        part[(long)blockIdx.x * 2 * D + threadIdx.x] = (red[threadIdx.x] + red[2 * D + threadIdx.x]) + (red[4 * D + threadIdx.x] + red[6 * D + threadIdx.x]);
-}
+    __shared__ __attribute__((aligned(16))) unsigned char smem[4 * BWD_WAVE_LDS + 2 * D * 4];
+    bwd_walk<0>(qkv, ld, out, ldo, dout, lddo, lse, dqkv, lddq, q_scale, k_scale, cosT, sinT, mask, part, d, smem);
+}
+
+#ifdef TATTN_ABLATION
+template <int ABL> __global__ __launch_bounds__(256, 2) void tattn16_fwd_abl(const bf16_t* __restrict__ qkv, int ld, bf16_t* __restrict__ out,
+                                                                            int ldo, float* __restrict__ lse, const float* __restrict__ q_scale,
+                                                                            const float* __restrict__ k_scale, const float* __restrict__ cosT,
+                                                                            const float* __restrict__ sinT, const uint8_t* __restrict__ mask, Dims d)
+{
+    __shared__ __attribute__((aligned(16))) unsigned char smem[4 * IMG];
+    fwd_walk<ABL>(qkv, ld, out, ldo, lse, q_scale, k_scale, cosT, sinT, mask, d, smem);
+}
+template <int ABL> __global__ __launch_bounds__(256, 2) void tattn16_bwd_abl(const bf16_t* __restrict__ qkv, int ld, const bf16_t* __restrict__ out,
+                                                                            int ldo, const bf16_t* __restrict__ dout, int lddo,
+                                                                            const float* __restrict__ lse, bf16_t* __restrict__ dqkv, int lddq,
+                                                                            const float* __restrict__ q_scale, const float* __restrict__ k_scale,
+                                                                            const float* __restrict__ cosT, const float* __restrict__ sinT,
+                                                                            const uint8_t* __restrict__ mask, float* __restrict__ part, Dims d)
+{
+    __shared__ __attribute__((aligned(16))) unsigned char smem[4 * BWD_WAVE_LDS + 2 * D * 4];
+    bwd_walk<ABL>(qkv, ld, out, ldo, dout, lddo, lse, dqkv, lddq, q_scale, k_scale, cosT, sinT, mask, part, d, smem);
+}
+int g_ablate = 0;
+#define TATTN_ABL_CASES(X) X(1) X(2) X(4) X(8) X(6) X(7) X(14) X(15)
+#endif
 
 int g_enable = 1;
-
-inline int bwd_blocks(long items) { return (int)((items + 3) / 4); }
+constexpr int DEFAULT_CAP = 512;
+int g_fwd_cap = DEFAULT_CAP, g_bwd_cap = DEFAULT_CAP;
+
+inline int grid_blocks(long items, int cap) { const long b = (items + 3) / 4; return (int)(b < cap ? b : cap); }
 
 bool shape_ok(int T_, int D_, int ld, int ldo, int dtype) {
     return g_enable && dtype == VVAE_DT_BF16 && T_ == T && D_ == D && ld % 8 == 0 && ldo % 8 == 0;
@@ -404,16 +568,42 @@
     return 0;
 }
 
+extern "C" int vvae_temporal_attn_mfma_config(int fwd_cap, int bwd_cap)
+{
+    tmfma::g_fwd_cap = fwd_cap > 0 ? fwd_cap : tmfma::DEFAULT_CAP;
+    tmfma::g_bwd_cap = bwd_cap > 0 ? bwd_cap : tmfma::DEFAULT_CAP;
+    return 0;
+}
+
+#ifdef TATTN_ABLATION
+extern "C" int vvae_tattn16_ablate(int bits)
+{
+    tmfma::g_ablate = bits & 15;
+    return 0;
+}
+#endif
+
 int tmfma_supported(int T, int D, int ld, int ldo, int dtype) { return tmfma::shape_ok(T, D, ld, ldo, dtype) ? 1 : 0; }
-int tmfma_bwd_rows(long items) { return tmfma::bwd_blocks(items); }
+int tmfma_bwd_rows(long items) { return tmfma::grid_blocks(items, tmfma::g_bwd_cap); }
 
 int tmfma_fwd(const void* qkv, int ld, void* out, int ldo, float* lse, const float* qs, const float* ks, const float* cosT, const float* sinT,
               const uint8_t* mask, int mask_div, int inner, int A, int heads, float eps, hipStream_t s)
 {
     tmfma::Dims d{A, heads, mask_div, inner, eps, (long)A * heads};
-    if (mask && ((uintptr_t)mask % 4)) return VVAE_ERR_BAD_ARG;
-    hipLaunchKernelGGL(tmfma::tattn16_fwd_mfma, dim3((unsigned)((d.items + 3) / 4)), dim3(256), 0, s, (const bf16_t*)qkv, ld, (bf16_t*)out, ldo, lse,
-                       qs, ks, cosT, sinT, mask, d);
+    if ((mask && ((uintptr_t)mask % 4)) || d.items > 0x7fffffffL) return VVAE_ERR_BAD_ARG;
+    const dim3 grid((unsigned)tmfma::grid_blocks(d.items, tmfma::g_fwd_cap));
+#ifdef TATTN_ABLATION
+#define X(B)                                                                                                                                \
+    if (tmfma::g_ablate == B) {                                                                                                             \
+        hipLaunchKernelGGL(tmfma::tattn16_fwd_abl<B>, grid, dim3(256), 0, s, (const bf16_t*)qkv, ld, (bf16_t*)out, ldo, lse, qs, ks, cosT,  \
+                           sinT, mask, d);                                                                                                  \
+        VVAE_LAUNCH_CHECK();                                                                                                                \
+        return 0;                                                                                                                           \
+    }
+    TATTN_ABL_CASES(X)
+#undef X
+#endif
+    hipLaunchKernelGGL(tmfma::tattn16_fwd_mfma, grid, dim3(256), 0, s, (const bf16_t*)qkv, ld, (bf16_t*)out, ldo, lse, qs, ks, cosT, sinT, mask, d);
     VVAE_LAUNCH_CHECK();
     return 0;
 }
@@ -423,9 +613,21 @@
               float* part, int A, int heads, float eps, hipStream_t s)
 {
     tmfma::Dims d{A, heads, mask_div, inner, eps, (long)A * heads};
-    if (mask && ((uintptr_t)mask % 4)) return VVAE_ERR_BAD_ARG;
-    hipLaunchKernelGGL(tmfma::tattn16_bwd_mfma, dim3((unsigned)tmfma::bwd_blocks(d.items)), dim3(256), 0, s, (const bf16_t*)qkv, ld,
-                       (const bf16_t*)out, ldo, (const bf16_t*)dout, lddo, lse, (bf16_t*)dqkv, lddq, qs, ks, cosT, sinT, mask, part, d);
+    if ((mask && ((uintptr_t)mask % 4)) || d.items > 0x7fffffffL) return VVAE_ERR_BAD_ARG;
+    const dim3 grid((unsigned)tmfma::grid_blocks(d.items, tmfma::g_bwd_cap));
+#ifdef TATTN_ABLATION
+#define X(B)                                                                                                                                \
+    if (tmfma::g_ablate == B) {                                                                                                             \
+        hipLaunchKernelGGL(tmfma::tattn16_bwd_abl<B>, grid, dim3(256), 0, s, (const bf16_t*)qkv, ld, (const bf16_t*)out, ldo,               \
+                           (const bf16_t*)dout, lddo, lse, (bf16_t*)dqkv, lddq, qs, ks, cosT, sinT, mask, part, d);                         \
+        VVAE_LAUNCH_CHECK();                                                                                                                \
+        return 0;                                                                                                                           \
+    }
+    TATTN_ABL_CASES(X)
+#undef X
+#endif
+    hipLaunchKernelGGL(tmfma::tattn16_bwd_mfma, grid, dim3(256), 0, s, (const bf16_t*)qkv, ld, (const bf16_t*)out, ldo, (const bf16_t*)dout, lddo,
+                       lse, (bf16_t*)dqkv, lddq, qs, ks, cosT, sinT, mask, part, d);
     VVAE_LAUNCH_CHECK();
     return 0;
 }
```
